# yell/boltzmann-machines

Hardware: AMD Instinct MI355X
Metric: Gibbs-steps/sec (CD-k, 784x1024 RBM, batch 512) (higher is better)
Workload: dtype f32

## Files before the change

### boltzmann_machines_amd/_ffi.py

```python
import ctypes as C
import os

import numpy as np

from . import build as _build

MAX_LAYERS = 4
UNIT_BERNOULLI, UNIT_GAUSSIAN, UNIT_MULTINOMIAL = 0, 1, 2


class Bm355Error(RuntimeError):
    pass


class RbmConfig(C.Structure):
    _fields_ = [('n_visible', C.c_int32), ('n_hidden', C.c_int32), ('v_unit', C.c_int32),
                ('sample_v_states', C.c_int32), ('sample_h_states', C.c_int32),
                ('dbm_first', C.c_int32), ('dbm_last', C.c_int32), ('max_batch', C.c_int32),
                ('l2', C.c_float), ('sparsity_target', C.c_float), ('sparsity_cost', C.c_float),
                ('sparsity_damping', C.c_float), ('dropout', C.c_float),
                ('h_unit', C.c_int32), ('n_samples', C.c_int32)]


class DbmConfig(C.Structure):
# ... 31 lines not shown
    'bm_rbm_set_grad_slot': [_vp, _i32],
    'bm_rbm_allreduce_grads_async': [_vp, _vp],
    'bm_rbm_wait_grads': [_vp, _i32],
    'bm_dbm_allreduce_grads': [_vp, _vp],
    'bm_xchg_create': [C.c_int32, C.c_int32, _vp, _sz, C.POINTER(_vp)],
    'bm_xchg_blob_bytes': [],
    'bm_xchg_export': [_vp, _vp],
    'bm_xchg_attach': [_vp, _vp],
    'bm_xchg_destroy': [_vp],
    'bm_xchg_allreduce_sum': [_vp, _vp],
    'bm_xchg_allreduce_max1': [_vp, _vp, _vp],
    'bm_xchg_status': [_vp, C.POINTER(C.c_int32)],
    'bm_xchg_info': [_vp, C.POINTER(C.c_int32), C.POINTER(C.c_int32), C.POINTER(_sz)],
    'bm_rbm_xchg_create': [_vp, C.c_int32, C.c_int32, C.POINTER(_vp)],
    'bm_dbm_xchg_create': [_vp, C.c_int32, C.c_int32, C.POINTER(_vp)],
    'bm_rbm_allreduce_grads_direct': [_vp, _vp],
    'bm_dbm_allreduce_grads_direct': [_vp, _vp],
    'bm_rbm_exchange_apply_direct': [_vp, _vp, _i32, C.c_float, C.c_float],
    'bm_rbm_exchange_gather_dw': [_vp, _vp],
    'bm_dbm_exchange_apply_ok': [_vp, _vp, C.POINTER(_i32)],
    'bm_dbm_exchange_apply_direct': [_vp, _vp, _i32, _i32, C.c_float, C.c_float],
    'bm_dbm_exchange_gather_dw': [_vp, _vp],
    'bm_xchg_set_timeout': [_vp, C.c_double],
    'bm_xchg_set_max_workgroups': [_vp, _i32],
    'bm_dbm_set_xchg': [_vp, _vp],
    'bm_dbm_set_fast_binary': [_vp, _i32],
    'bm_dbm_set_ais_literal': [_vp, _i32],
    'bm_dbm_set_sigmoid_literal': [_vp, _i32],
    'bm_rbm_set_fast_binary': [_vp, _i32],
    'bm_rbm64_create': [C.POINTER(RbmConfig), C.POINTER(C.c_double), C.POINTER(_vp)],
    'bm_rbm64_destroy': [_vp],
    'bm_rbm64_sync': [_vp],
    'bm_rbm64_seed': [_vp, C.c_uint64],
    'bm_rbm64_set_row_offset': [_vp, C.c_int64],
    'bm_rbm64_set_param': [_vp, C.c_char_p, _vp, _sz],
    'bm_rbm64_get_param': [_vp, C.c_char_p, _vp, _sz],
    'bm_rbm64_train_step': [_vp, _vp, C.c_int32, C.c_double, C.c_double, C.c_int32],
    'bm_rbm64_train_step_metrics': [_vp, _vp, C.c_int32, C.c_double, C.c_double, C.c_int32, C.POINTER(C.c_double)],
    'bm_rbm64_transform': [_vp, _vp, C.c_int32, C.c_int32, _vp],
    'bm_rbm64_metrics': [_vp, _vp, C.c_int32, C.c_int32, C.POINTER(C.c_double)],
    'bm_rbm64_free_energy': [_vp, _vp, C.c_int32, C.POINTER(C.c_double)],
    'bm_dbm64_create': [C.POINTER(DbmConfig), C.POINTER(C.c_double), C.POINTER(_vp)],
    'bm_dbm64_destroy': [_vp],
    'bm_dbm64_sync': [_vp],
    'bm_dbm64_seed': [_vp, C.c_uint64],
    'bm_dbm64_set_row_offset': [_vp, C.c_int64, C.c_int64],
    'bm_dbm64_set_param': [_vp, C.c_char_p, _vp, _sz],
    'bm_dbm64_get_param': [_vp, C.c_char_p, _vp, _sz],
    'bm_dbm64_train_step': [_vp, _vp, C.c_double, C.c_double, C.c_int32, C.POINTER(C.c_int32), C.POINTER(C.c_double)],
    'bm_dbm64_metrics': [_vp, _vp, C.c_int32, C.POINTER(C.c_int32), C.POINTER(C.c_double)],
    'bm_dbm64_mean_field': [_vp, _vp, _vp, C.POINTER(C.c_int32)],
    'bm_dbm64_reconstruct': [_vp, _vp, _vp],
    'bm_dbm64_sample_v': [_vp, C.c_int32, _vp],
    'bm_dbm64_ais': [_vp, C.c_int32, C.c_int32, C.c_int32, C.c_uint64, C.c_int64, _vp],
    'bm_dbm64_log_proba': [_vp, _vp, _vp],
    'bm_rbm_create': [C.POINTER(RbmConfig), C.POINTER(_vp)],
    'bm_rbm_destroy': [_vp],
    'bm_rbm_sync': [_vp],
    'bm_rbm_set_param': [_vp, C.c_char_p, _vp, _sz],
    'bm_rbm_get_param': [_vp, C.c_char_p, _vp, _sz],
    'bm_rbm_set_param_dev': [_vp, C.c_char_p, _vp, _sz],
    'bm_rbm_dev_ptr': [_vp, C.c_char_p, C.POINTER(_vp), C.POINTER(_sz)],
    'bm_rbm_seed': [_vp, _u64],
    'bm_rbm_set_row_offset': [_vp, _i64],
    'bm_rbm_train_step': [_vp, _vp, _i32, _f32, _f32, _i32],
    'bm_rbm_train_step_metrics': [_vp, _vp, _i32, _f32, _f32, _i32, _fp],
    'bm_rbm_train_step_metrics_async': [_vp, _vp, _i32, _f32, _f32, _i32],
    'bm_rbm_collect_metrics': [_vp, _fp, _i32, C.POINTER(C.c_int32)],
    'bm_rbm_train_epoch': [_vp, _vp, _i64, _i32, _f32, _f32, _i32],
    'bm_rbm_stage': [_vp, _i32],
    'bm_rbm_get_staged': [_vp, _i32, C.c_char_p, _vp, _sz],
    'bm_rbm_grad_step': [_vp, _vp, _i32, _i32],
    'bm_rbm_apply_step': [_vp, _i32, _f32, _f32],
    'bm_rbm_transform': [_vp, _vp, _i32, _i32, _vp],
    'bm_rbm_metrics': [_vp, _vp, _i32, _i32, _fp],
    'bm_rbm_free_energy': [_vp, _vp, _i32, _fp],
    'bm_rbm_free_energy_rows': [_vp, _vp, _i32, _vp],
    'bm_rbm_ais': [_vp, _i32, _i32, _i32, _vp, _u64, _i64, _vp],
    'bm_rbm_gibbs': [_vp, _vp, _vp, _i32, _i32],
    'bm_rbm_stream': [_vp, C.POINTER(_vp)],
    'bm_rbm_profile': [_vp, _i32],
    'bm_rbm_kernel_times': [_vp, _fp, _ip],
    'bm_rbm_chain_stats': [_vp, C.POINTER(C.c_int64)],
    'bm_rbm_timer_start': [_vp],
    'bm_rbm_timer_stop': [_vp, _fp],
    'bm_rbm_timer_mark': [_vp],
    'bm_rbm_timer_elapsed': [_vp, _fp],
    'bm_dbm_create': [C.POINTER(DbmConfig), C.POINTER(_vp)],
    'bm_dbm_destroy': [_vp],
    'bm_dbm_sync': [_vp],
    'bm_dbm_seed': [_vp, _u64],
    'bm_dbm_set_row_offset': [_vp, _i64, _i64],
    'bm_dbm_set_param': [_vp, C.c_char_p, _vp, _sz],
    'bm_dbm_get_param': [_vp, C.c_char_p, _vp, _sz],
    'bm_dbm_dev_ptr': [_vp, C.c_char_p, C.POINTER(_vp), C.POINTER(_sz)],
    'bm_dbm_train_step': [_vp, _vp, _f32, _f32, _i32, _ip, _fp],
    'bm_dbm_metrics': [_vp, _vp, _i32, _ip, _fp],
    'bm_dbm_grad_step': [_vp, _vp, _i32, _ip],
    'bm_dbm_apply_step': [_vp, _i32, _i32, _f32, _f32],
    'bm_dbm_set_mf_allreduce': [_vp, _vp, _vp],
    'bm_dbm_set_comm': [_vp, _vp],
    'bm_dbm_ais_sharded': [_vp, _vp, _i32, _i32, _i32, _u64, _vp],
    'bm_dbm_ais_sharded_direct': [_vp, _vp, _i32, _i32, _i32, _u64, _vp],
    'bm_dbm_stream': [_vp, C.POINTER(_vp)],
    'bm_dbm_mean_field': [_vp, _vp, _vp, _ip],
    'bm_dbm_reconstruct': [_vp, _vp, _vp],
    'bm_dbm_sample_v': [_vp, _i32, _vp],
    'bm_dbm_ais': [_vp, _i32, _i32, _i32, _u64, _i64, _vp],
    'bm_dbm_log_proba': [_vp, _vp, _vp],
    'bm_dbm_timer_start': [_vp],
    'bm_dbm_timer_stop': [_vp, _fp],
    'bm_dbm_timer_mark': [_vp],
    'bm_dbm_timer_elapsed': [_vp, _fp],
}
_RESTYPE = {'bm_last_error': C.c_char_p, 'bm_version': C.c_char_p}
MF_REDUCE_FN = C.CFUNCTYPE(C.c_float, C.c_float, C.c_void_p)

_lib = None


def load(rebuild=True):
    global _lib
    if _lib is not None:
        return _lib
    path = _build.LIB
    if rebuild and _build.needs_build():
        import shutil
        have_hipcc = bool(shutil.which('hipcc')) or os.path.exists('/opt/rocm/bin/hipcc')
        try:
            _build.build()
        except Exception as e:
            if have_hipcc or not os.path.exists(path):
                raise Bm355Error('libbm355.so could not be built from the current sources: %s' % e)
            import warnings
            warnings.warn('libbm355.so is older than its sources and hipcc is not available; using the existing '
                          'library (%s)' % e)
    if not os.path.exists(path):
        raise Bm355Error('libbm355.so not found at %s (run __graft_entry__.build())' % path)
    lib = C.CDLL(path)
    for name, restype in _RESTYPE.items():
        f = getattr(lib, name)
        f.restype = restype
        f.argtypes = []
    for name, argtypes in SIGNATURES.items():
        f = getattr(lib, name)
        f.restype = C.c_int
        f.argtypes = argtypes
    _lib = lib
    return lib


def check(rc):
    if rc != 0:
        raise Bm355Error(load().bm_last_error().decode('utf-8', 'replace'))


def exported_symbols():
    return sorted(list(SIGNATURES) + list(_RESTYPE))


class DeviceArray(object):

    def __init__(self, shape, dtype=np.float32, ptr=None, owner=None):
        self.shape = tuple(int(s) for s in (shape if hasattr(shape, '__iter__') else (shape,)))
        self.dtype = np.dtype(dtype)
        self.nbytes = int(np.prod(self.shape)) * self.dtype.itemsize
# ... 52 lines not shown
```

### boltzmann_machines_amd/csrc/bm_chain.h

```cpp
#pragma once
#include "bm_kernels.h"

namespace bm {

constexpr int CHAIN_MAXPH = 24;
constexpr int CHAIN_MAXTI = 64;
using GeoChain = GeoAct8;

struct ChainPhase {
    Operand P, Q; int K; int p_xm; int I;
    const float *bias, *sigma;
    float mult, bmult; int kind, sample;
    float *means, *states, *negmeans; int ldo;
    PhiloxKey key; long long row0;
};

struct ChainArgs {
    int nph, J, tiles_j, rounds_cap, dbg;
    unsigned gen;
    unsigned *flags;
    unsigned *claim;
    unsigned *claim_zero;
    int *status;
    long long *stamps;
// ... 88 lines not shown
    while (true) {
        const int r = small_div(n, T);
        if (r >= R) break;
        const int rem = n - r * T;
        int p = 0;
#pragma unroll
        for (int q = 1; q < CHAIN_MAXPH; ++q) p += (q < c.nph && rem >= c.tp0[q]) ? 1 : 0;
        const int ti = rem - c.tp0[p];
        unsigned nxt = 0;
        const ChainPhase &ph = c.ph[p];
        ActArgs a;
        a.P1 = ph.P; a.Q1 = ph.Q; a.K1 = ph.K; a.p_xm = ph.p_xm;
        a.P2 = Operand{nullptr, 0, 0, 0}; a.Q2 = a.P2; a.K2 = 0;
        a.I = ph.I; a.J = c.J;
        a.bias = ph.bias; a.sigma = ph.sigma; a.mult = ph.mult; a.bmult = ph.bmult; a.kind = ph.kind; a.sample = ph.sample;
        a.means = ph.means; a.states = ph.states; a.negmeans = ph.negmeans; a.ldo = ph.ldo;
        a.key = ph.key; a.row0 = ph.row0;
        a.prev = nullptr; a.maxdiff = nullptr; a.maxdiff_blk = nullptr;
        a.rowacc = nullptr; a.beta_a = 0.f; a.beta_b = 0.f; a.rowacc_single = 0; a.rowdot_out = nullptr; a.ld_part = 0;
        a.dot_vec = nullptr; a.dot_mat = nullptr; a.ld_dot = 0;
        a.acc_init = nullptr; a.ld_init = 0; a.skip = nullptr;
        a.chk_ctl = nullptr; a.chk_slots = nullptr; a.chk_n = 0; a.chk_tol = 0.f;
        a.b3 = Bf3Range{}; a.states16 = nullptr; a.ld16 = 0; a.map_xi = 0;
        a.fe_rowacc2 = nullptr; a.fe_flip = nullptr; a.fe_x = nullptr; a.fe_ldx = 0; a.fe_w = nullptr; a.fe_ldw = 0;
        a.fe_zero = nullptr; a.fe_rm = 0; a.fe_key = PhiloxKey{0u, 0u, 0u, 0u};
#ifdef BM_PROBE
        a.dbg = nullptr;
#endif
        unsigned *fl = c.flags + ((size_t)(team * c.rounds_cap + r) * CHAIN_MAXPH) * CHAIN_MAXTI;
        const unsigned *wfl = (p > 0 && !(c.dbg & 2)) ? fl + (size_t)(p - 1) * CHAIN_MAXTI : nullptr;
        const int nwait = p > 0 ? c.tp0[p] - c.tp0[p - 1] : 0;
        const int tj = team + 8 * r;
        long long *stp = c.stamps ? c.stamps + ((size_t)blockIdx.x * 16 + (ntiles < 15 ? ntiles : 15)) * 8 : nullptr;
        if (stp && tid == 0) { stp[0] = wall_clock64(); stp[5] = (long long)p; stp[6] = (long long)ti; stp[7] = (long long)team; }
        if (ph.p_xm) chain_tile<G, XM, COH>(a, ti * G::TI, tj * G::TJ, smem, wfl, nwait, c.gen, c.status, stp, c.dbg & 4, my_claim, nxt);
        else         chain_tile<G, KM, COH>(a, ti * G::TI, tj * G::TJ, smem, wfl, nwait, c.gen, c.status, stp, c.dbg & 4, my_claim, nxt);
        asm volatile("s_waitcnt vmcnt(0)" ::: "memory");
        if (tid == 0) s_claim = nxt;
        wg_barrier();
        if (tid == 0) __hip_atomic_store(fl + (size_t)p * CHAIN_MAXTI + ti, c.gen, __ATOMIC_RELAXED, __HIP_MEMORY_SCOPE_AGENT);
        if (stp && tid == 0) stp[4] = wall_clock64();
        n = (int)s_claim;
        ++ntiles;
    }
    if (tid == 0 && ntiles) atomicAdd(c.status + 1, ntiles);
}

struct ChainState {
    unsigned *flags = nullptr, *claim = nullptr;
    int *status = nullptr;
    int rounds_cap = 0;
    unsigned gen = 0;
    unsigned launches = 0;
    long long tiles_expected = 0;
    bool on = false;
    int mode = -1;
    int ncu = 0;
    std::vector<ActArgs> rec;
    std::vector<Operand> alt_p;
    long long *stamps = nullptr;
    static constexpr int CLAIM_SLOTS = 16;
    static constexpr size_t STAMP_WORDS = 256 * 16 * 8;
    ChainState() = default;
    ChainState(const ChainState &) = delete;
    ChainState &operator=(const ChainState &) = delete;
    ~ChainState() { release(); }
    void release() {
        if (stamps) {
            const char *f = bm::dbg("chain_stamps");
            std::vector<long long> hst(STAMP_WORDS);
            if (f && hipMemcpy(hst.data(), stamps, STAMP_WORDS * 8, hipMemcpyDeviceToHost) == hipSuccess) {
                FILE *fp = fopen(f, "wb");
                if (fp) { fwrite(hst.data(), 8, STAMP_WORDS, fp); fclose(fp); }
            }
            (void)hipFree(stamps); stamps = nullptr;
        }
        if (flags) (void)hipFree(flags);
        if (claim) (void)hipFree(claim);
        if (status) (void)hipFree(status);
        flags = claim = nullptr; status = nullptr;
    }
};

static inline int chain_mode(ChainState &cs) {
    if (cs.mode < 0) {
        const char *e = bm::dbg("chain");
        cs.mode = e ? atoi(e) : 1;
        hipDeviceProp_t pr; int d = 0, nxcc = 0; (void)hipGetDevice(&d);
        const bool have = hipGetDeviceProperties(&pr, d) == hipSuccess;
        cs.ncu = have ? pr.multiProcessorCount : 0;
        if (hipDeviceGetAttribute(&nxcc, hipDeviceAttributeNumberOfXccs, d) != hipSuccess) nxcc = 0;
        const bool arch = have && (strncmp(pr.gcnArchName, "gfx950", 6) == 0 || strncmp(pr.gcnArchName, "gfx942", 6) == 0);
        if (!(arch && nxcc == 8 && cs.ncu == 256)) cs.mode = 0;
    }
    return cs.mode;
}

static inline bool chain_phase_ok(const ActArgs &a) {
    using G = GeoChain;
    if (a.K2 > 0 || a.b3.K1 > 0 || a.prev || a.maxdiff || a.maxdiff_blk || a.rowacc || a.rowdot_out || a.acc_init ||
        a.skip || a.chk_ctl || a.states16 || a.dot_mat || a.fe_flip) return false;
    if (a.kind != 0 && a.kind != 1) return false;
    const int pl = a.p_xm ? XM : KM;
    if (!(operand_fast(a.P1, pl, a.K1) && operand_fast(a.Q1, XM, a.K1))) return false;
    if (a.K1 < G::PF * G::BK) return false;
    if ((a.I + G::TI - 1) / G::TI > CHAIN_MAXTI) return false;
    return true;
}

static inline int chain_flush(ChainState &cs, hipStream_t st, int maxB) {
    cs.on = false;
    std::vector<ActArgs> rec;
    std::vector<Operand> alt;
    rec.swap(cs.rec);
    alt.swap(cs.alt_p);
    if (rec.empty()) return 0;
    alt.resize(rec.size(), Operand{nullptr, 0, 0, 0});
    using G = GeoChain;
    bool ok = chain_mode(cs) > 0 && rec.size() >= (cs.mode == 1 ? 6u : 2u);
    const int J = rec[0].J, tiles_j = (J + G::TJ - 1) / G::TJ;
    for (const ActArgs &a : rec) ok = ok && chain_phase_ok(a) && a.J == J;
    if (ok && cs.mode == 1) {
        ok = tiles_j >= 8;
        for (const ActArgs &a : rec) ok = ok && ((a.I + G::TI - 1) / G::TI) * ((tiles_j + 7) / 8) <= 2 * 32;
    }
    if (!ok) {
        for (size_t i = 0; i < rec.size(); ++i) {
            if (alt[i].ptr) { rec[i].P1 = alt[i]; rec[i].p_xm = 1; }
            launch_act(rec[i], st);
        }
        return 0;
    }
    const int rounds = (tiles_j + 7) / 8;
    if (!cs.flags || rounds > cs.rounds_cap) {
        if (cs.flags) { if (hipStreamSynchronize(st) != hipSuccess) return -1; (void)hipFree(cs.flags); cs.flags = nullptr; }
        const int cap = std::max(rounds, ((maxB + G::TJ - 1) / G::TJ + 7) / 8);
        const size_t nfl = (size_t)8 * cap * CHAIN_MAXPH * CHAIN_MAXTI;
        if (hipMalloc((void **)&cs.flags, nfl * 4) != hipSuccess) return -1;
        if (hipMemsetAsync(cs.flags, 0, nfl * 4, st) != hipSuccess) return -1;
        cs.rounds_cap = cap;
        cs.gen = 0;
        if (!cs.claim) {
            if (hipMalloc((void **)&cs.claim, (size_t)ChainState::CLAIM_SLOTS * 8 * 32 * 4) != hipSuccess) return -1;
            if (hipMemsetAsync(cs.claim, 0, (size_t)ChainState::CLAIM_SLOTS * 8 * 32 * 4, st) != hipSuccess) return -1;
            if (hipMalloc((void **)&cs.status, 2 * sizeof(int)) != hipSuccess) return -1;
            if (hipMemsetAsync(cs.status, 0, 2 * sizeof(int), st) != hipSuccess) return -1;
        }
    }
    for (size_t first = 0; first < rec.size(); first += CHAIN_MAXPH) {
        const int nph = (int)std::min<size_t>(CHAIN_MAXPH, rec.size() - first);
        ChainArgs c;
        memset(&c, 0, sizeof(c));
        c.nph = nph; c.J = J; c.tiles_j = tiles_j; c.rounds_cap = cs.rounds_cap;
        if (++cs.gen == 0) {
            if (hipMemsetAsync(cs.flags, 0, (size_t)8 * cs.rounds_cap * CHAIN_MAXPH * CHAIN_MAXTI * 4, st) != hipSuccess) return -1;
            cs.gen = 1;
        }
        c.gen = cs.gen;
        c.flags = cs.flags;
        c.claim = cs.claim + (size_t)(cs.launches % ChainState::CLAIM_SLOTS) * 8 * 32;
        c.claim_zero = cs.claim + (size_t)((cs.launches + ChainState::CLAIM_SLOTS / 2) % ChainState::CLAIM_SLOTS) * 8 * 32;
        ++cs.launches;
        c.status = cs.status;
        int tiles = 0;
        for (int p = 0; p < nph; ++p) {
            const ActArgs &a = rec[first + p];
            ChainPhase &ph = c.ph[p];
            ph.P = a.P1; ph.Q = a.Q1; ph.K = a.K1; ph.p_xm = a.p_xm; ph.I = a.I;
            ph.bias = a.bias; ph.sigma = a.sigma; ph.mult = a.mult; ph.bmult = a.bmult; ph.kind = a.kind; ph.sample = a.sample;
            ph.means = a.means; ph.states = a.states; ph.negmeans = a.negmeans; ph.ldo = a.ldo;
            ph.key = a.key; ph.row0 = a.row0;
            c.tp0[p] = tiles;
            tiles += (a.I + G::TI - 1) / G::TI;
        }
        for (int p = nph; p <= CHAIN_MAXPH; ++p) c.tp0[p] = tiles;
        cs.tiles_expected += (long long)tiles * tiles_j;
// ... 13 lines not shown
```

### boltzmann_machines_amd/csrc/bm_gemm.h

```cpp
#pragma once
#include <hip/hip_runtime.h>
#include <stdint.h>
#include <stdlib.h>
#include <string.h>

namespace bm {

struct NoSide {
    static constexpr bool kFinalSync = true;
    static constexpr bool kSplitFill = false, kCohQ = false;
    static constexpr bool kCanAbort = false;
    __device__ __forceinline__ void wait_inputs() {}
    __device__ __forceinline__ void post_fill() {}
    __device__ __forceinline__ void fill() {}
    __device__ __forceinline__ void drain() {}
};

#define BM_ABL(bit) ((ABL >> (bit)) & 1)

typedef float f32x4 __attribute__((ext_vector_type(4)));
typedef float f32x2v __attribute__((ext_vector_type(2)));

constexpr int NT = 256;

enum : int { KM = 0, XM = 1 };

template <int WI_, int WJ_, int MI_, int NJ_, int BK_, int NB_ = 4>
struct Geo {
    static constexpr int WI = WI_, WJ = WJ_, MI = MI_, NJ = NJ_, BK = BK_;
    static constexpr int NBUF = NB_;
    static constexpr int PF = NB_ - 1;
    static constexpr int NW = WI * WJ;
    static constexpr int NT = 64 * NW;
    static constexpr int TI = 16 * MI * WI;
    static constexpr int TJ = 16 * NJ * WJ;
    static constexpr int E = 4 * MI;
    static constexpr int P_BUF = TI * BK;
    static constexpr int Q_BUF = TJ * BK;
    static constexpr int SMEM_FLOATS = NBUF * (P_BUF + Q_BUF);
    static constexpr int NPP = P_BUF * 4 / (1024 * NW);
    static constexpr int NPQ = Q_BUF * 4 / (1024 * NW);
    static constexpr int NVP = TI * BK / (4 * NT);
    static constexpr int NVQ = TJ * BK / (4 * NT);
    static constexpr int SP = (MI == 2) ? 8 : 4;
    static constexpr int SQ = (NJ == 2) ? 8 : 4;
    static_assert(MI == 1 || MI == 2, "MI");
    static_assert(NJ == 1 || NJ == 2, "NJ");
    static_assert(BK == 32 || BK == 64, "BK");
    static_assert(NB_ >= 4 && NB_ <= 8, "ring depth");
    static_assert(NPP >= 1 && NPP * 1024 * NW == P_BUF * 4, "P chunk must split into whole DMA pieces per wave");
    static_assert(NPQ >= 1 && NPQ * 1024 * NW == Q_BUF * 4, "Q chunk must split into whole DMA pieces per wave");
    static_assert(NVP >= 1 && NVP * 4 * NT == TI * BK && NVQ >= 1 && NVQ * 4 * NT == TJ * BK, "register path split");
    static_assert(SMEM_FLOATS * 4 <= 160 * 1024 - 1024, "LDS");
};
using GeoAct = Geo<2, 2, 2, 1, 64>;
using GeoAct8 = Geo<2, 4, 1, 1, 64>;
using GeoActS = Geo<2, 2, 1, 1, 64>;
using GeoActS32 = Geo<2, 2, 1, 1, 32>;
using GeoAct32 = Geo<2, 2, 2, 1, 32>;
using GeoGrad = Geo<2, 2, 2, 2, 64>;
using GeoGrad8 = Geo<2, 4, 2, 1, 64>;
using GeoGrad8h = Geo<2, 4, 2, 1, 32>;
using GeoBf3S = Geo<1, 4, 2, 1, 64>;

struct Operand {
    const float *ptr;
    int ld;
    int nx;
    int vec;
};

static inline Operand make_operand(const float *p, int ld, int nx) {
    Operand o;
    o.ptr = p; o.ld = ld; o.nx = nx;
    o.vec = (((uintptr_t)p & 15u) == 0 && (ld & 3) == 0) ? 1 : 0;
    return o;
}

static inline bool operand_fast(const Operand &o, int layout, int K) {
    if (!o.ptr) return true;
    if (!o.vec) return false;
    return layout == KM ? (o.nx % 4 == 0 && o.nx >= 4) : (K % 4 == 0);
}

template <int BK> __device__ __forceinline__ int fx(int row) { return (BK == 64) ? (row & 15) : ((row >> 1) & 7); }
template <int S> __device__ __forceinline__ int fk(int row) { return S * ((row >> 2) & 1); }

template <int L, int TX, int BK, int S>
__device__ __forceinline__ int img_off(int row, int c4) {
    return (L == XM) ? row * BK + ((c4 ^ fx<BK>(row)) << 2) : row * TX + ((c4 ^ fk<S>(row)) << 2);
}

__device__ __forceinline__ float4 load4_guard(const float *p, bool row_ok, int col, int ncols, bool vec) {
    float4 v = make_float4(0.f, 0.f, 0.f, 0.f);
    if (row_ok) {
// ... 150 lines not shown
}

template <class G, int ABL = 0>
__device__ __forceinline__ void mfma_frags_head(f32x4 (&acc)[G::MI][G::NJ], const Frags<G> &f, int nq) {
#pragma unroll
    for (int q = 0; q < G::BK / 16; ++q) {
        if (q < nq) {
#pragma unroll
            for (int kk = 4 * q; kk < 4 * q + 4; ++kk) {
#pragma unroll
                for (int n = 0; n < G::NJ; ++n) {
                    const float qv = f.q[kk][n];
#pragma unroll
                    for (int t = 0; t < G::MI; ++t) {
                        if (BM_ABL(1)) { acc[t][n][0] += f.p[kk][t] * qv; continue; }
                        acc[t][n] = __builtin_amdgcn_mfma_f32_16x16x4f32(f.p[kk][t], qv, acc[t][n], 0, 0, 0);
                    }
                }
            }
        }
    }
}

template <class G> struct ChunkRegs {
    float4 p[G::NVP];
    float4 q[G::NVQ];
};

struct KRange {
    Operand P1, Q1; int K1;
    Operand P2, Q2; int K2;
};

__device__ __forceinline__ int sel_i(int a, int b, int m) { return a ^ ((a ^ b) & m); }
__device__ __forceinline__ const float *sel_p(const float *a, const float *b, int m) {
    const uintptr_t ua = (uintptr_t)a, ub = (uintptr_t)b;
    return (const float *)(ua ^ ((ua ^ ub) & (uintptr_t)(intptr_t)m));
}

template <class G, int DW = G::NW> struct DmaPlan {
    static constexpr int NPP = G::P_BUF / (256 * DW), NPQ = G::Q_BUF / (256 * DW);
    uint32_t p[NPP], q[NPQ];
};

template <int L, int TX, int BK, int NW, int NP, int S>
__device__ __forceinline__ void plan_offsets(uint32_t (&off)[NP], int ld, int nx, int x0, int wave, int lane) {
    constexpr int RC = (L == KM) ? TX / 4 : BK / 4;
    constexpr int R = 64 / RC;
#pragma unroll
    for (int n = 0; n < NP; ++n) {
        const int pc = wave + n * NW;
        const int row = pc * R + lane / RC, slot = lane % RC;
        if (L == KM) {
            const int c4 = slot ^ fk<S>(row);
            off[n] = (uint32_t)(row * ld + min(x0 + c4 * 4, nx - 4)) * 4u;
        } else {
            const int c4 = slot ^ fx<BK>(row);
            off[n] = (uint32_t)(min(x0 + row, nx - 1) * ld + c4 * 4) * 4u;
        }
    }
}

template <int QL, class G, int PL = KM, int DW = G::NW>
__device__ __forceinline__ void make_plan(DmaPlan<G, DW> &pl, const Operand &P, const Operand &Q, int i0, int j0, int wave, int lane) {
    plan_offsets<PL, G::TI, G::BK, DW, DmaPlan<G, DW>::NPP, G::SP>(pl.p, P.ld, P.nx, i0, wave, lane);
    plan_offsets<QL, G::TJ, G::BK, DW, DmaPlan<G, DW>::NPQ, G::SQ>(pl.q, Q.ld, Q.nx, j0, wave, lane);
}

__device__ __forceinline__ void dma16(const char *src, float *lds_dst) {
    unsigned keep;
    const unsigned lds_addr = (unsigned)(uintptr_t)(__attribute__((address_space(3))) void *)lds_dst;
    asm volatile("s_mov_b32 %0, m0\n\ts_mov_b32 m0, %2\n\ts_nop 0\n\tglobal_load_lds_dwordx4 %1, off\n\ts_mov_b32 m0, %0"
                 : "=&s"(keep) : "v"(src), "s"(__builtin_amdgcn_readfirstlane(lds_addr)) : "memory");
}

__device__ __forceinline__ void dma16s(const void *sbase, uint32_t voff, unsigned lds_byte) {
    asm volatile("s_mov_b32 m0, %2\n\ts_nop 0\n\tglobal_load_lds_dwordx4 %1, %0"
                 :: "s"(sbase), "v"(voff), "s"(lds_byte) : "memory");
}
__device__ __forceinline__ void dma16s_coh(const void *sbase, uint32_t voff, unsigned lds_byte) {
    asm volatile("s_mov_b32 m0, %2\n\ts_nop 0\n\tglobal_load_lds_dwordx4 %1, %0 sc1"
                 :: "s"(sbase), "v"(voff), "s"(lds_byte) : "memory");
}
template <class G, int DW, bool QSC = false, bool QHALF = false>
__device__ __forceinline__ void dma_chunk_s(const DmaPlan<G, DW> &pl, const char *pb, const char *qb, unsigned ldsP, unsigned ldsQ) {
#pragma unroll
    for (int n = 0; n < DmaPlan<G, DW>::NPP; ++n) dma16s(pb, pl.p[n], ldsP + (unsigned)(n * DW * 1024));
#pragma unroll
    for (int n = 0; n < DmaPlan<G, DW>::NPQ; ++n) {
        if (QHALF && (n & 1)) continue;
        if (QSC) dma16s_coh(qb, pl.q[n], ldsQ + (unsigned)(n * DW * 1024));
        else     dma16s(qb, pl.q[n], ldsQ + (unsigned)(n * DW * 1024));
    }
}

template <int QL, class G, bool SEG2, int PL = KM, int DW = G::NW, bool QHALF = false>
__device__ __forceinline__ void dma_chunk(const KRange &kr, const DmaPlan<G, DW> &pl1, const DmaPlan<G, DW> &pl2, int nch1, int c,
                                          float *sP, float *sQ, int wave) {
    constexpr int BK = G::BK;
    const int m = SEG2 ? -(int)(c >= nch1) : 0;
    const int kc = c - (nch1 & m);
    const int ldp = SEG2 ? sel_i(kr.P1.ld, kr.P2.ld, m) : kr.P1.ld;
    const int ldq = SEG2 ? sel_i(kr.Q1.ld, kr.Q2.ld, m) : kr.Q1.ld;
    const char *pb = (const char *)((SEG2 ? sel_p(kr.P1.ptr, kr.P2.ptr, m) : kr.P1.ptr) +
                                    ((PL == KM) ? (size_t)kc * BK * ldp : (size_t)kc * BK));
    const char *qb = (const char *)((SEG2 ? sel_p(kr.Q1.ptr, kr.Q2.ptr, m) : kr.Q1.ptr) +
                                    ((QL == KM) ? (size_t)kc * BK * ldq : (size_t)kc * BK));
#pragma unroll
    for (int n = 0; n < DmaPlan<G, DW>::NPP; ++n) {
        const uint32_t o1 = pl1.p[n], o2 = SEG2 ? pl2.p[n] : 0u;
        const uint32_t o = SEG2 ? (o1 ^ ((o1 ^ o2) & (uint32_t)m)) : o1;
        dma16(pb + o, sP + (wave + n * DW) * 256);
    }
#pragma unroll
    for (int n = 0; n < DmaPlan<G, DW>::NPQ; ++n) {
        if (QHALF && (n & 1)) continue;
        const uint32_t o1 = pl1.q[n], o2 = SEG2 ? pl2.q[n] : 0u;
        const uint32_t o = SEG2 ? (o1 ^ ((o1 ^ o2) & (uint32_t)m)) : o1;
        dma16(qb + o, sQ + (wave + n * DW) * 256);
    }
}

template <int QL, class G, bool FAST, bool SEG2, int PL = KM, bool COHQ = false>
__device__ __forceinline__ void load_chunk(ChunkRegs<G> &r, const KRange &kr, int nch1, int i0, int j0, int c, int tid) {
    constexpr int BK = G::BK;
    if (!SEG2) {
        g2r<PL, G::TI, BK, G::NT, FAST>(r.p, kr.P1.ptr, kr.P1.ld, kr.P1.nx, kr.P1.vec, i0, c * BK, kr.K1, tid);
        g2r<QL, G::TJ, BK, G::NT, FAST, COHQ>(r.q, kr.Q1.ptr, kr.Q1.ld, kr.Q1.nx, kr.Q1.vec, j0, c * BK, kr.K1, tid);
    } else {
        const int m = -(int)((c >= nch1) & (kr.K2 > 0));
        const int kc = c - (nch1 & m);
        const int K = sel_i(kr.K1, kr.K2, m);
        g2r<PL, G::TI, BK, G::NT, FAST>(r.p, sel_p(kr.P1.ptr, kr.P2.ptr, m), sel_i(kr.P1.ld, kr.P2.ld, m),
                                        sel_i(kr.P1.nx, kr.P2.nx, m), sel_i(kr.P1.vec, kr.P2.vec, m), i0, kc * BK, K, tid);
        g2r<QL, G::TJ, BK, G::NT, FAST, COHQ>(r.q, sel_p(kr.Q1.ptr, kr.Q2.ptr, m), sel_i(kr.Q1.ld, kr.Q2.ld, m),
                                              sel_i(kr.Q1.nx, kr.Q2.nx, m), sel_i(kr.Q1.vec, kr.Q2.vec, m), j0, kc * BK, K, tid);
    }
}

template <int QL, class G, bool SEG2, int PL = KM>
__device__ __forceinline__ void store_chunk(const ChunkRegs<G> &r, const KRange &kr, int nch1, int c,
                                            float *sP, float *sQ, int tid) {
    constexpr int BK = G::BK;
    const int m = SEG2 ? -(int)((c >= nch1) & (kr.K2 > 0)) : 0;
    const int kz = sel_i(kr.K1, kr.K2, m) - (c - (nch1 & m)) * BK;
    r2s<PL, G::TI, BK, G::NT, G::SP>(r.p, sP, tid, kz);
    r2s<QL, G::TJ, BK, G::NT, G::SQ>(r.q, sQ, tid, kz);
}

template <class G> struct RegPlan {
    uint32_t p[G::NVP], q[G::NVQ];
};
template <int L, int TX, int BK, int NTH>
__device__ __forceinline__ void reg_offsets(uint32_t (&off)[TX * BK / (4 * NTH)], int ld, int nx, int x0, int tid) {
    constexpr int NV = TX * BK / (4 * NTH);
    constexpr int RC = (L == KM) ? TX / 4 : BK / 4;
#pragma unroll
    for (int n = 0; n < NV; ++n) {
        const int f = tid + n * NTH;
        const int row = f / RC, c4 = f % RC;
        off[n] = (L == KM) ? (uint32_t)(row * ld + min(x0 + c4 * 4, nx - 4)) * 4u
                           : (uint32_t)(min(x0 + row, nx - 1) * ld + c4 * 4) * 4u;
    }
}
template <int QL, class G, int PL = KM>
__device__ __forceinline__ void make_reg_plan(RegPlan<G> &pl, const Operand &P, const Operand &Q, int i0, int j0, int tid) {
    reg_offsets<PL, G::TI, G::BK, G::NT>(pl.p, P.ld, P.nx, i0, tid);
    reg_offsets<QL, G::TJ, G::BK, G::NT>(pl.q, Q.ld, Q.nx, j0, tid);
}
template <int QL, class G, bool SEG2, int PL = KM>
__device__ __forceinline__ void load_chunk_slim(ChunkRegs<G> &r, const KRange &kr, const RegPlan<G> &pl1,
                                                const RegPlan<G> &pl2, int nch1, int c) {
    constexpr int BK = G::BK;
    const int m = SEG2 ? -(int)(c >= nch1) : 0;
    const int kc = c - (nch1 & m);
    const int ldp = SEG2 ? sel_i(kr.P1.ld, kr.P2.ld, m) : kr.P1.ld;
    const int ldq = SEG2 ? sel_i(kr.Q1.ld, kr.Q2.ld, m) : kr.Q1.ld;
    const char *pb = (const char *)((SEG2 ? sel_p(kr.P1.ptr, kr.P2.ptr, m) : kr.P1.ptr) +
                                    ((PL == KM) ? (size_t)kc * BK * ldp : (size_t)kc * BK));
    const char *qb = (const char *)((SEG2 ? sel_p(kr.Q1.ptr, kr.Q2.ptr, m) : kr.Q1.ptr) +
                                    ((QL == KM) ? (size_t)kc * BK * ldq : (size_t)kc * BK));
#pragma unroll
    for (int n = 0; n < G::NVP; ++n) {
        const uint32_t o1 = pl1.p[n], o2 = SEG2 ? pl2.p[n] : 0u;
        const uint32_t o = SEG2 ? (o1 ^ ((o1 ^ o2) & (uint32_t)m)) : o1;
        r.p[n] = *reinterpret_cast<const float4 *>(pb + o);
    }
#pragma unroll
    for (int n = 0; n < G::NVQ; ++n) {
        const uint32_t o1 = pl1.q[n], o2 = SEG2 ? pl2.q[n] : 0u;
        const uint32_t o = SEG2 ? (o1 ^ ((o1 ^ o2) & (uint32_t)m)) : o1;
        r.q[n] = *reinterpret_cast<const float4 *>(qb + o);
    }
}
template <int QL, class G, int PL = KM>
__device__ __forceinline__ void store_chunk_slim(const ChunkRegs<G> &r, float *sP, float *sQ, int tid) {
    r2s<PL, G::TI, G::BK, G::NT, G::SP, false>(r.p, sP, tid, 0);
    r2s<QL, G::TJ, G::BK, G::NT, G::SQ, false>(r.q, sQ, tid, 0);
}

enum : int { STG_DMA = 0, STG_REG = 1, STG_DMAH = 2 };

#define BM_WAIT_VM(n) asm volatile("s_waitcnt vmcnt(%0)" ::"n"(n) : "memory")
template <int NPW, int MAXC>
__device__ __forceinline__ void wait_vm_chunks(int n) {
    static_assert(MAXC * NPW <= 63, "vmcnt range");
    if (MAXC >= 4 && n >= 4)      BM_WAIT_VM(4 * NPW <= 63 ? 4 * NPW : 0);
    else if (MAXC >= 3 && n == 3) BM_WAIT_VM(3 * NPW <= 63 ? 3 * NPW : 0);
    else if (MAXC >= 2 && n == 2) BM_WAIT_VM(2 * NPW <= 63 ? 2 * NPW : 0);
    else if (n == 1)              BM_WAIT_VM(NPW);
    else                          BM_WAIT_VM(0);
}
__device__ __forceinline__ void wg_barrier() {
    asm volatile("s_waitcnt lgkmcnt(0)" ::: "memory");
    __builtin_amdgcn_s_barrier();
    asm volatile("" ::: "memory");
}

template <int QL, class G, bool FAST, bool SEG2, int ABL = 0, int PL = KM, int STG = STG_DMA, class Side = NoSide>
__device__ __forceinline__ void mainloop(f32x4 (&acc)[G::MI][G::NJ], const KRange &kr, int i0, int j0, float *smem,
                                         Side &side, long long *stamps = nullptr) {
#ifdef BM_PROBE
#define BM_MSTAMP(n) do { if (stamps && threadIdx.x == 0) stamps[n] = (long long)__builtin_readcyclecounter(); } while (0)
#else
#define BM_MSTAMP(n) do {} while (0)
#endif
    constexpr int BK = G::BK, P_BUF = G::P_BUF, Q_BUF = G::Q_BUF, NBUF = G::NBUF, PF = G::PF;
    constexpr int DW = (STG == STG_DMAH && G::NW == 8) ? 4 : G::NW;
    constexpr int NPW = DmaPlan<G, DW>::NPP + (BM_ABL(9) ? (DmaPlan<G, DW>::NPQ + 1) / 2 : DmaPlan<G, DW>::NPQ);
    const int tid = threadIdx.x, lane = tid & 63;
    const int w = __builtin_amdgcn_readfirstlane(tid >> 6);
    const int wi = w % G::WI, wj = w / G::WI;
    float *sP = smem, *sQ = smem + NBUF * P_BUF;
    const int nch1 = (kr.K1 + BK - 1) / BK;
    const int nch = nch1 + (SEG2 ? (kr.K2 + BK - 1) / BK : 0);
    const int nfull1 = kr.K1 / BK, nfull2 = SEG2 ? kr.K2 / BK : 0;
    auto is_full = [&](int c) -> bool {
        return (c < nfull1) | (SEG2 && c >= nch1 && c - nch1 < nfull2);
    };
    auto is_dma = [&](int c) -> bool {
        if (!FAST || STG == STG_REG || BM_ABL(6)) return false;
        return is_full(c);
    };
    ChunkRegs<G> gr;
    Frags<G> fa, fb;
    DmaPlan<G, DW> pl1, pl2;
    RegPlan<G> rp1, rp2;
    const bool dmaw = (DW == G::NW) || w < DW;
    ChunkRegs<G> g0, g1;
    if (FAST && STG != STG_REG && dmaw) {
        make_plan<QL, G, PL, DW>(pl1, kr.P1, kr.Q1, i0, j0, w, lane);
        if (SEG2) make_plan<QL, G, PL, DW>(pl2, kr.P2, kr.Q2, i0, j0, w, lane);
    }
    int n_reg = 0;
    if (FAST && STG == STG_REG && !BM_ABL(6) && !BM_ABL(0)) {
        while (n_reg + 4 < nch && is_full(n_reg + 4) && is_full(n_reg + 2)) ++n_reg;
        n_reg &= ~1;
        if (n_reg > 0 && !(is_full(0) && is_full(1) && is_full(2) && is_full(3))) n_reg = 0;
        if (n_reg > 0) {
            make_reg_plan<QL, G, PL>(rp1, kr.P1, kr.Q1, i0, j0, tid);
            if (SEG2) make_reg_plan<QL, G, PL>(rp2, kr.P2, kr.Q2, i0, j0, tid);
        }
    }
    BM_MSTAMP(0);
    if (n_reg > 0) {
        ChunkRegs<G> ga, gb;
        load_chunk_slim<QL, G, SEG2, PL>(ga, kr, rp1, rp2, nch1, 0);
        load_chunk_slim<QL, G, SEG2, PL>(gb, kr, rp1, rp2, nch1, 1);
        load_chunk_slim<QL, G, SEG2, PL>(g0, kr, rp1, rp2, nch1, 2);
        load_chunk_slim<QL, G, SEG2, PL>(g1, kr, rp1, rp2, nch1, 3);
        __builtin_amdgcn_sched_barrier(0);
        side.fill();
        __builtin_amdgcn_sched_barrier(0);
        store_chunk_slim<QL, G, PL>(ga, sP, sQ, tid);
        store_chunk_slim<QL, G, PL>(gb, sP + P_BUF, sQ + Q_BUF, tid);
    } else if constexpr (Side::kSplitFill) {
        static_assert(FAST && STG == STG_DMA && DW == G::NW, "chained fill");
        const unsigned l0 = (unsigned)(uintptr_t)(__attribute__((address_space(3))) void *)smem;
        const unsigned lP = l0 + (unsigned)w * 1024u, lQ = l0 + (unsigned)(NBUF * P_BUF * 4) + (unsigned)w * 1024u;
#pragma unroll
        for (int c = 0; c < PF; ++c) {
            const char *pb = (const char *)kr.P1.ptr + (size_t)c * ((PL == KM) ? (size_t)BK * kr.P1.ld * 4 : (size_t)BK * 4);
#pragma unroll
            for (int n = 0; n < DmaPlan<G, DW>::NPP; ++n) dma16s(pb, pl1.p[n], lP + (unsigned)(c * P_BUF * 4 + n * DW * 1024));
        }
        __builtin_amdgcn_sched_barrier(0);
        side.fill();
        __builtin_amdgcn_sched_barrier(0);
        side.wait_inputs();
#pragma unroll
        for (int c = 0; c < PF; ++c) {
            const char *qb = (const char *)kr.Q1.ptr + (size_t)c * ((QL == KM) ? (size_t)BK * kr.Q1.ld * 4 : (size_t)BK * 4);
#pragma unroll
            for (int n = 0; n < DmaPlan<G, DW>::NPQ; ++n) dma16s_coh(qb, pl1.q[n], lQ + (unsigned)(c * Q_BUF * 4 + n * DW * 1024));
        }
        constexpr int NQ_LEFT = (PF - 2) * DmaPlan<G, DW>::NPQ;
        BM_WAIT_VM(NQ_LEFT);
    } else {
#pragma unroll
        for (int c = 0; c < PF; ++c)
            if (c < nch && is_dma(c) && dmaw && !BM_ABL(0))
                dma_chunk<QL, G, SEG2, PL, DW, (BM_ABL(9) != 0)>(kr, pl1, pl2, nch1, c, sP + (c % NBUF) * P_BUF, sQ + (c % NBUF) * Q_BUF, w);
        __builtin_amdgcn_sched_barrier(0);
        side.fill();
        __builtin_amdgcn_sched_barrier(0);
#pragma unroll
        for (int c = 0; c < 2; ++c)
            if (c < nch && !is_dma(c) && !BM_ABL(0)) {
                load_chunk<QL, G, FAST, SEG2, PL>(gr, kr, nch1, i0, j0, c, tid);
                store_chunk<QL, G, SEG2, PL>(gr, kr, nch1, c, sP + (c % NBUF) * P_BUF, sQ + (c % NBUF) * Q_BUF, tid);
            }
        {
            int n_after = 0;
#pragma unroll
            for (int c = 2; c < PF; ++c) n_after += (c < nch && is_dma(c) && !BM_ABL(0)) ? 1 : 0;
            wait_vm_chunks<NPW, PF - 2>(n_after);
        }
    }
    BM_MSTAMP(1);
    if (!BM_ABL(5)) wg_barrier();
    if constexpr (Side::kCanAbort) {
        side.post_fill();
        if (side.aborted) { BM_WAIT_VM(0); return; }
    }
    read_frags<QL, G, ABL, PL>(fa, sP, sQ, wi, wj, lane);
    BM_MSTAMP(2);
    const int klast = (SEG2 && kr.K2 > 0) ? kr.K2 - (nch - nch1 - 1) * BK : kr.K1 - (nch1 - 1) * BK;
    const int nq_last = (klast + 15) / 16;
    constexpr int NM = (BK / 4) * G::MI * G::NJ;
    constexpr int NRP = (PL == XM) ? BK / 16 : BK / 4;
    constexpr int NRQ = (QL == XM) ? (BK / 16) * G::NJ : BK / 4;
    constexpr int NR = NRP + NRQ;
#define BM_SG(mask, n) __builtin_amdgcn_sched_group_barrier(mask, n, 0);
#ifndef BM_SCHED_VARIANT
#define BM_SCHED_VARIANT 0
#endif
#if BM_SCHED_VARIANT == 0
#define BM_SCHED_STEP                                                                             \
    if (DW == G::NW) { _Pragma("unroll") for (int s_ = 0; s_ < NPW; ++s_) { BM_SG(0x008, 1) BM_SG(0x020, 1) } } \
    _Pragma("unroll") for (int s_ = 0; s_ < NR; ++s_) { BM_SG(0x008, 1) BM_SG(0x100, 1) }         \
    BM_SG(0x008, NM)
#elif BM_SCHED_VARIANT == 1
#define BM_SCHED_STEP                                                                             \
    _Pragma("unroll") for (int s_ = 0; s_ < NR; ++s_) { BM_SG(0x008, 1) BM_SG(0x100, 1) }         \
    _Pragma("unroll") for (int s_ = 0; s_ < NPW; ++s_) { BM_SG(0x008, 1) BM_SG(0x020, 1) }        \
    BM_SG(0x008, NM)
#else
#define BM_SCHED_STEP
#endif
    static_assert(NBUF == 4, "the steps below are written for a 4-slot ring");
    int cc = 0;
    const unsigned lds0 = (unsigned)(uintptr_t)(__attribute__((address_space(3))) void *)smem;
    const unsigned ldsPw = lds0 + (unsigned)w * 1024u, ldsQw = lds0 + (unsigned)(NBUF * P_BUF * 4) + (unsigned)w * 1024u;
    bool in2 = false;
    auto chunk_bases = [&](int c, const char *&pb, const char *&qb) {
        const bool s2 = SEG2 && c >= nch1;
        const Operand &P = s2 ? kr.P2 : kr.P1, &Q = s2 ? kr.Q2 : kr.Q1;
        const int kc = s2 ? c - nch1 : c;
        pb = (const char *)P.ptr + (size_t)kc * ((PL == KM) ? (size_t)BK * P.ld * 4 : (size_t)BK * 4);
        qb = (const char *)Q.ptr + (size_t)kc * ((QL == KM) ? (size_t)BK * Q.ld * 4 : (size_t)BK * 4);
    };
#define BM_DMA_AT(CD, SD)                                                                         \
    {                                                                                             \
        if (SEG2 && !in2 && (CD) >= nch1) { in2 = true; pl1 = pl2; }                              \
        const char *pb_, *qb_;                                                                    \
        chunk_bases((CD), pb_, qb_);                                                              \
        if (dmaw) dma_chunk_s<G, DW, Side::kCohQ, (BM_ABL(9) != 0)>(pl1, pb_, qb_, ldsPw + (unsigned)((SD) * P_BUF * 4), \
                                     ldsQw + (unsigned)((SD) * Q_BUF * 4));                       \
    }
#define BM_STEP_Q(FC, FN, S)                                                                      \
    {                                                                                             \
        BM_DMA_AT(cc + PF, ((S) + PF) % NBUF)                                                     \
        read_frags<QL, G, ABL, PL>(FN, sP + (((S) + 1) % NBUF) * P_BUF, sQ + (((S) + 1) % NBUF) * Q_BUF, wi, wj, lane); \
        mfma_frags<G, ABL>(acc, FC);                                                              \
        BM_SCHED_STEP                                                                             \
        if (!BM_ABL(8)) BM_WAIT_VM((PF - 2) * NPW);                                               \
        if (!BM_ABL(5)) wg_barrier();                                                             \
        ++cc;                                                                                     \
    }
#define BM_STEP_T(FC, FN, S1, S2, S3)       \
    {                                                                                             \
        const int cd = cc + PF, cr = cc + 2;                                                      \
        const bool do_dma = cd < nch && is_dma(cd) && !BM_ABL(0);                                 \
        const bool do_reg = cr < nch && !is_dma(cr) && !BM_ABL(0);                                \
        if (cc == last - 1) side.drain();       \
        if (do_reg) load_chunk<QL, G, FAST, SEG2, PL, Side::kCohQ>(gr, kr, nch1, i0, j0, cr, tid); \
        if (do_dma) BM_DMA_AT(cd, S3)                                                             \
        read_frags<QL, G, ABL, PL>(FN, sP + (S1) * P_BUF, sQ + (S1) * Q_BUF, wi, wj, lane);       \
        mfma_frags<G, ABL>(acc, FC);                                                              \
        _Pragma("unroll") for (int s_ = 0; s_ < NR; ++s_) { BM_SG(0x008, 1) BM_SG(0x100, 1) }     \
        BM_SG(0x008, NM)                                                                          \
        if (do_reg) {                                                                             \
            BM_WAIT_VM(0);                                                                        \
            store_chunk<QL, G, SEG2, PL>(gr, kr, nch1, cr, sP + (S2) * P_BUF, sQ + (S2) * Q_BUF, tid); \
        } else if (cr < nch) {                                                                    \
             \
            int n_after = 0;                                                                      \
            _Pragma("unroll") for (int c_ = 3; c_ <= PF; ++c_) n_after += (cc + c_ < nch && is_dma(cc + c_) && !BM_ABL(0)) ? 1 : 0; \
            wait_vm_chunks<NPW, PF - 2>(n_after);                                                 \
        }                                                                                         \
        if (!BM_ABL(5)) wg_barrier();                                                             \
        ++cc;                                                                                     \
    }
#define BM_STEP_TC(FC, FN, S) BM_STEP_T(FC, FN, ((S) + 1) % NBUF, ((S) + 2) % NBUF, ((S) + 3) % NBUF)
#define BM_STEP_TR(FC, FN)    BM_STEP_T(FC, FN, (cc + 1) % NBUF, (cc + 2) % NBUF, (cc + 3) % NBUF)
    constexpr int NWR = G::NVP + G::NVQ;
#ifndef BM_REG_SCHED_VARIANT
#define BM_REG_SCHED_VARIANT 0
#endif
#if BM_REG_SCHED_VARIANT == 0
#define BM_REG_SCHED(RELOAD)                                                                      \
        _Pragma("unroll") for (int s_ = 0; s_ < NWR; ++s_) { BM_SG(0x008, 1) BM_SG(0x200, 1) }    \
        if (RELOAD) { _Pragma("unroll") for (int s_ = 0; s_ < NWR; ++s_) { BM_SG(0x008, 1) BM_SG(0x020, 1) } } \
        _Pragma("unroll") for (int s_ = 0; s_ < NR; ++s_) { BM_SG(0x008, 1) BM_SG(0x100, 1) }     \
        BM_SG(0x008, NM)
#elif BM_REG_SCHED_VARIANT == 1
#define BM_REG_SCHED(RELOAD)                                                                      \
        _Pragma("unroll") for (int s_ = 0; s_ < NR; ++s_) { BM_SG(0x008, (NM >= 64 ? 2 : 1)) BM_SG(0x100, 2) } \
        _Pragma("unroll") for (int s_ = 0; s_ < NWR; ++s_) { BM_SG(0x008, (NM >= 32 ? 2 : 1)) BM_SG(0x200, 1) } \
        if (RELOAD) { _Pragma("unroll") for (int s_ = 0; s_ < NWR; ++s_) { BM_SG(0x008, 1) BM_SG(0x020, 1) } } \
        BM_SG(0x008, NM)
#else
#define BM_REG_SCHED(RELOAD)
#endif
#define BM_STEP_REG(FC, FN, G_, RELOAD, S)                                                        \
    {                                                                                             \
        store_chunk_slim<QL, G, PL>(G_, sP + (((S) + 2) % NBUF) * P_BUF, sQ + (((S) + 2) % NBUF) * Q_BUF, tid); \
        if (RELOAD) load_chunk_slim<QL, G, SEG2, PL>(G_, kr, rp1, rp2, nch1, cc + 4);             \
        read_frags<QL, G, ABL, PL>(FN, sP + (((S) + 1) % NBUF) * P_BUF, sQ + (((S) + 1) % NBUF) * Q_BUF, wi, wj, lane); \
        mfma_frags<G, ABL>(acc, FC);                                                              \
        BM_REG_SCHED(RELOAD)                                                                      \
        if (!BM_ABL(5)) wg_barrier();                                                             \
        ++cc;                                                                                     \
    }
    if (n_reg > 0) {
        int left = n_reg;
#pragma unroll 1
        while (left >= 4) {
            BM_STEP_REG(fa, fb, g0, true, 0)
            BM_STEP_REG(fb, fa, g1, true, 1)
            BM_STEP_REG(fa, fb, g0, true, 2)
            BM_STEP_REG(fb, fa, g1, true, 3)
            left -= 4;
        }
        if (left == 2) {
            BM_STEP_REG(fa, fb, g0, true, 0)
            BM_STEP_REG(fb, fa, g1, true, 1)
            BM_STEP_REG(fa, fb, g0, false, 2)
            BM_STEP_REG(fb, fa, g1, false, 3)
        } else {
            BM_STEP_REG(fa, fb, g0, false, 0)
            BM_STEP_REG(fb, fa, g1, false, 1)
        }
    }
    int n_steady = 0;
    if (FAST && STG != STG_REG && !BM_ABL(6) && !BM_ABL(0))
        while (n_steady + PF < nch) {
            bool all = true;
#pragma unroll
            for (int c_ = 2; c_ <= PF; ++c_) all = all && is_dma(n_steady + c_);
            if (!all) break;
            ++n_steady;
        }
#pragma unroll 1
    for (int q = 0; q < n_steady / 4; ++q) {
        BM_STEP_Q(fa, fb, 0)
        BM_STEP_Q(fb, fa, 1)
        BM_STEP_Q(fa, fb, 2)
        BM_STEP_Q(fb, fa, 3)
// ... 170 lines not shown
```

### boltzmann_machines_amd/csrc/bm_kernels.h

```cpp
#pragma once
#include <stdio.h>
#include <stdlib.h>
#include <string.h>
#include "bm_gemm.h"
#include "bm_bf3.h"
#include "bm_numerics.h"
#include "bm_rng.h"

namespace bm {

struct MfCtl { unsigned maxdiff; int done; int steps; float resid; };

struct ActArgs {
    Operand P1, Q1; int K1;
    int p_xm;
    Operand P2, Q2; int K2;
    int I, J;
    const float *bias;
    const float *sigma;
    float mult;
    float bmult;
    int kind;
    int sample;
    int lit;
// ... 44 lines not shown
    uint32_t w[4];
    philox_block(key, idx >> 2, w);
    return (int)(w[idx & 3] % (uint32_t)V);
}
#define FE_FLIP_FROM_KEY (reinterpret_cast<const int *>(uintptr_t(1)))
constexpr int BM_MF_SLOTS = 1024;

__device__ __forceinline__ void draw4(const ActArgs &a, const PhiloxKey &key, unsigned long long flat, int ib, int nvalid,
                                      const float *m, float *s, bool aligned) {
    if (aligned) {
        uint32_t wds[4];
        philox_block(key, flat >> 2, wds);
        if (a.kind == 0) {
#pragma unroll
            for (int r = 0; r < 4; ++r) s[r] = (u32_to_uniform(wds[r]) < m[r]) ? 1.f : 0.f;
        } else {
            float n[4];
            box_muller(wds[0], wds[1], n[0], n[1]);
            box_muller(wds[2], wds[3], n[2], n[3]);
#pragma unroll
            for (int r = 0; r < 4; ++r) s[r] = n[r] * a.sigma[ib + r] + m[r];
        }
    } else {
#pragma unroll
        for (int r = 0; r < 4; ++r) {
            if (r >= nvalid) break;
            const unsigned long long idx = flat + r;
            uint32_t wds[4];
            philox_block(key, idx >> 2, wds);
            if (a.kind == 0) {
                s[r] = (u32_to_uniform(wds[idx & 3]) < m[r]) ? 1.f : 0.f;
            } else {
                float n0, n1;
                const int pr = (int)(idx & 3) >> 1;
                box_muller(wds[2 * pr], wds[2 * pr + 1], n0, n1);
                s[r] = ((idx & 1) ? n1 : n0) * a.sigma[ib + r] + m[r];
            }
        }
    }
}

#ifndef BM_NT_STORES
#define BM_NT_STORES 1
#endif
typedef float f32x2 __attribute__((ext_vector_type(2)));
__device__ __forceinline__ void stream_store4(float *p, float x, float y, float z, float w) {
    if (BM_NT_STORES) __builtin_nontemporal_store((f32x4){x, y, z, w}, reinterpret_cast<f32x4 *>(p));
    else *reinterpret_cast<float4 *>(p) = make_float4(x, y, z, w);
}
__device__ __forceinline__ void stream_store2(float *p, float x, float y) {
    if (BM_NT_STORES) __builtin_nontemporal_store((f32x2){x, y}, reinterpret_cast<f32x2 *>(p));
    else *reinterpret_cast<float2 *>(p) = make_float2(x, y);
}

template <bool CACHED = false>
__device__ __forceinline__ void store4(float *dst, size_t o, const float *v, int nvalid, bool v4) {
    if (v4) {
        if (CACHED) *reinterpret_cast<float4 *>(dst + o) = make_float4(v[0], v[1], v[2], v[3]);
        else stream_store4(dst + o, v[0], v[1], v[2], v[3]);
    } else {
#pragma unroll
        for (int r = 0; r < 4; ++r) if (r < nvalid) dst[o + r] = v[r];
    }
}

template <int MI> struct PhiloxFor { typedef PhiloxPair type; };
template <> struct PhiloxFor<1> { typedef PhiloxOne type; };

__device__ __forceinline__ float wave_max_lane63(float v) {
#define BM_DPP_MAX(ctrl, rmask) v = fmaxf(v, __int_as_float(__builtin_amdgcn_update_dpp(__float_as_int(v), __float_as_int(v), ctrl, rmask, 0xf, false)))
    BM_DPP_MAX(0xb1, 0xf);
    BM_DPP_MAX(0x4e, 0xf);
    BM_DPP_MAX(0x124, 0xf);
    BM_DPP_MAX(0x128, 0xf);
    BM_DPP_MAX(0x142, 0xa);
    BM_DPP_MAX(0x143, 0xc);
#undef BM_DPP_MAX
    return v;
}

template <int E, class Rng, bool MF = false, int NTH = 256> struct ActSide {
    static constexpr bool kFinalSync = false;
    static constexpr bool kSplitFill = false, kCohQ = false, kCanAbort = MF;
    static constexpr bool kMF = MF;
    const float *bias, *sigma;
    const float *prev_row;
    int ib0, I, with_rng;
    float bs[E], sg[E], pv[E];
    Rng rng;
    MfCtl *chk_ctl; const float *chk_slots; int chk_n; float chk_tol; const int *skip; float *s_chk; int aborted, nthreads;

    __device__ __forceinline__ void load_inputs() {
        const float *sp = sigma ? sigma : bias;
        const bool has_sigma = sigma != nullptr;
        if (MF && prev_row) {
            if (E == 4 && ib0 + 3 < I && (((uintptr_t)prev_row & 15u) == 0)) {
                const float4 t = *reinterpret_cast<const float4 *>(prev_row);
                pv[0] = t.x; pv[1] = t.y; pv[2] = t.z; pv[E - 1] = t.w;
            } else {
#pragma unroll
                for (int e = 0; e < E; ++e) pv[e] = (ib0 + e < I) ? prev_row[e] : 0.f;
            }
        }
        if (MF && E == 4 && ib0 + 3 < I && (((uintptr_t)(bias + ib0) & 15u) == 0) && (((uintptr_t)(sp + ib0) & 15u) == 0)) {
            const float4 b = *reinterpret_cast<const float4 *>(bias + ib0), v = *reinterpret_cast<const float4 *>(sp + ib0);
            bs[0] = b.x; bs[1] = b.y; bs[2] = b.z; bs[E - 1] = b.w;
            sg[0] = has_sigma ? v.x : 1.0f; sg[1] = has_sigma ? v.y : 1.0f; sg[2] = has_sigma ? v.z : 1.0f; sg[E - 1] = has_sigma ? v.w : 1.0f;
            return;
        }
#pragma unroll
        for (int e = 0; e < E; ++e) {
            const int i = (ib0 + e < I) ? ib0 + e : I - 1;
            bs[e] = bias[i];
            const float sv = sp[i];
            sg[e] = has_sigma ? sv : 1.0f;
        }
    }
    static constexpr int CHK_MAX = 4096;
    float *s_slots;
    static __device__ __forceinline__ void dma4_lane0(const void *src, float *lds_dst) {
        if ((threadIdx.x & 63) == 0) {
            unsigned keep;
            const unsigned lds_addr = (unsigned)(uintptr_t)(__attribute__((address_space(3))) void *)lds_dst;
            asm volatile("s_mov_b32 %0, m0\n\ts_mov_b32 m0, %2\n\ts_nop 0\n\tglobal_load_lds_dword %1, off\n\ts_mov_b32 m0, %0"
                         : "=&s"(keep) : "v"(src), "s"(__builtin_amdgcn_readfirstlane(lds_addr)) : "memory");
        }
    }
    __device__ __forceinline__ void preload() {
        if constexpr (MF) {
            load_inputs();
            aborted = 0;
            const int w = threadIdx.x >> 6, lane = threadIdx.x & 63;
            if (chk_ctl) {
                for (int p = w; p * 256 < chk_n && p * 256 < CHK_MAX; p += nthreads / 64)
                    dma16(reinterpret_cast<const char *>(chk_slots + 256 * p) + 16 * lane, s_slots + 256 * p);
                if (w == 0) dma4_lane0(&chk_ctl->done, s_slots + CHK_MAX);
            } else if (skip) {
                if (w == 0) dma4_lane0(skip, s_slots + CHK_MAX);
            }
        }
    }
    __device__ __forceinline__ void fill() {
        if (!MF) load_inputs();
        if (with_rng) rng.fill();
    }
    __device__ __forceinline__ void post_fill() {
        if constexpr (MF) {
            if (chk_ctl) {
                constexpr int NR = CHK_MAX / (4 * NTH);
                f32x4 v[NR];
#pragma unroll
                for (int q = 0; q < NR; ++q) {
                    const int e = 4 * ((int)threadIdx.x + q * NTH);
                    v[q] = *reinterpret_cast<const f32x4 *>(s_slots + (e < chk_n ? e : 0));
                }
                float m = 0.f;
#pragma unroll
                for (int q = 0; q < NR; ++q) {
                    const bool in = 4 * ((int)threadIdx.x + q * NTH) < chk_n;
                    m = fmaxf(m, in ? fmaxf(fmaxf(v[q][0], v[q][1]), fmaxf(v[q][2], v[q][3])) : 0.f);
                }
                m = wave_max_lane63(m);
                if ((threadIdx.x & 63) == 63) s_chk[threadIdx.x >> 6] = m;
                wg_barrier();
                m = 0.f;
#pragma unroll
// ... 433 lines not shown
                    a.u.vb[c] = a.u.vb[c] + d;
                }
            }
        }
    } else {
        const int c0 = (wv - nv) * 64;
        block_colsum(a.h0m, a.ldh0, a.hm, a.ldh, c0, a.u.H, a.B, true, smem, s1, s2, a.hm_negated != 0);
        if ((lane & 15) == 0) {
#pragma unroll
            for (int r = 0; r < 4; ++r) {
                const int h = c0 + w * 16 + g * 4 + r;
                if (h < a.u.H) {
                    const float sq = s2[r];
                    a.raw_tail[a.u.V + h] = s1[r];
                    a.raw_tail[a.u.V + a.u.H + h] = sq;
                    if (a.raw_only) continue;
                    const float qn = a.u.damping * a.u.q[h] + (1.0f - a.u.damping) * sq;
                    a.u.q[h] = qn;
                    const float pen = a.u.cost * (qn - a.u.target);
                    a.u.pen[h] = pen;
                    float gr = s1[r] / a.u.N;
                    gr = gr - pen;
                    const float d = a.u.lr * (a.u.mom * a.u.dhb[h] + gr);
                    a.u.dhb[h] = d;
                    a.u.hb[h] = a.u.hb[h] + d;
                }
            }
        }
    }
}

__global__ __launch_bounds__(NT) void rbm_bias_fused_kernel(RbmBiasFusedArgs a) {
    __shared__ __attribute__((aligned(16))) float smem[CS_SMEM_FLOATS];
    rbm_bias_fused_block(a, blockIdx.x, smem);
}

struct GradArgs {
    Operand Ppos, Qpos; int Kpos;
    Operand Pneg, Qneg; int Kneg;
    int I, J;
    int form;
    int fused;
    float *raw;
    float *raw2;
    float *W, *dW;
    float *Wt;
    int ldw, ldwt;
    const float *pen;
    float N, M, l2, lr, mom;
    int nbias;
    RbmBiasFusedArgs bias;
    int fetch_at_fill;
    int map_xi;
#ifdef BM_PROBE
    long long *dbg;
#endif
};

__device__ __forceinline__ void apply_w_update(float g, float pen, float l2, float lr, float mom,
                                               float &w, float &dw) {
    g = __fsub_rn(g, __fmul_rn(l2, w));
    g = __fsub_rn(g, pen);
    const float d = __fmul_rn(lr, __fadd_rn(__fmul_rn(mom, dw), g));
    dw = d;
    w = __fadd_rn(w, d);
}
__device__ __forceinline__ bool grad_pow2(float N) { return ((__float_as_uint(N) & 0x007fffffu) == 0u) && N >= 1.0f; }
__device__ __forceinline__ float grad_norm1(float r, float N, float invN, bool pow2) {
    return pow2 ? __fmul_rn(r, invN) : __fdiv_rn(r, N);
}
__device__ __forceinline__ float grad_norm2(float r, float r2, float N, float M, float invN, float invM, bool pow2) {
    return pow2 ? __fsub_rn(__fmul_rn(r, invN), __fmul_rn(r2, invM)) : __fsub_rn(__fdiv_rn(r, N), __fdiv_rn(r2, M));
}

struct DivBy {
    float n, inv; bool pow2;
    __device__ __forceinline__ explicit DivBy(float N) : n(N), inv(1.0f / N),
        pow2(grad_pow2(N)) {}
};

template <int NJ> struct GradSide {
    static constexpr bool kFinalSync = true;
    static constexpr bool kSplitFill = false, kCohQ = false, kCanAbort = false;
    const float *W, *dW; int ldw, I, J, ib0, jb[NJ]; bool on, vec8;
    float4 w[NJ][2], d[NJ][2];
    bool at_fill;
    __device__ __forceinline__ void fill() { if (at_fill) fetch(); }
    __device__ __forceinline__ void drain() { if (!at_fill) fetch(); }
    __device__ __forceinline__ void fetch() {
        if (!on || ib0 >= I) return;
#pragma unroll
        for (int n = 0; n < NJ; ++n) {
            if (jb[n] >= J) continue;
            const size_t o = (size_t)jb[n] * ldw + ib0;
            if (vec8) {
                w[n][0] = *reinterpret_cast<const float4 *>(W + o);  w[n][1] = *reinterpret_cast<const float4 *>(W + o + 4);
                d[n][0] = *reinterpret_cast<const float4 *>(dW + o); d[n][1] = *reinterpret_cast<const float4 *>(dW + o + 4);
            } else {
                float tw[8], td[8];
#pragma unroll
                for (int e = 0; e < 8; ++e) {
                    const bool ok = ib0 + e < I;
                    tw[e] = ok ? W[o + e] : 0.f;
                    td[e] = ok ? dW[o + e] : 0.f;
                }
                w[n][0] = make_float4(tw[0], tw[1], tw[2], tw[3]); w[n][1] = make_float4(tw[4], tw[5], tw[6], tw[7]);
                d[n][0] = make_float4(td[0], td[1], td[2], td[3]); d[n][1] = make_float4(td[4], td[5], td[6], td[7]);
            }
        }
    }
};

template <class G, bool FAST, int ABL = 0, int STG = STG_DMA, int MINB = 1>
__global__ __launch_bounds__(G::NT, MINB) void grad_kernel(GradArgs a, TileMap tmap) {
    constexpr int TI = G::TI, NJ = G::NJ;
    static_assert(G::MI == 2 && G::TI == 64 && G::TJ == 64, "grad_kernel: 64 x 64 tiles, 8 consecutive outputs per lane");
    __shared__ __attribute__((aligned(16))) float smem[G::SMEM_FLOATS];
    constexpr bool kBias = G::SMEM_FLOATS >= CS_SMEM_FLOATS;
    static_assert(G::NT >= NT, "bias path");
    const int ntile_blocks = (int)gridDim.x - a.nbias;
    if ((int)blockIdx.x >= ntile_blocks) {
        if constexpr (kBias) {
            if (G::NT > NT && threadIdx.x >= NT) return;
            rbm_bias_fused_block(a.bias, (int)blockIdx.x - ntile_blocks, smem);
        }
        return;
    }
    asm volatile("" :: "s"(a.Ppos.ptr), "s"(a.Qpos.ptr), "s"(a.Ppos.ld), "s"(a.Qpos.ld), "s"(a.Ppos.nx), "s"(a.Qpos.nx),
                       "s"(a.Pneg.ptr), "s"(a.Qneg.ptr), "s"(a.Pneg.ld), "s"(a.Qneg.ld), "s"(a.Kpos), "s"(a.Kneg),
                       "s"(a.I), "s"(a.J), "s"(a.W), "s"(a.dW), "s"(a.ldw), "s"(a.form), "s"(a.fused));
    constexpr int TJ2 = G::TJ;
    int ti, tj;
    if (tmap.slab) {
        block_to_tile((a.J + TJ2 - 1) / TJ2, ti, tj, 0, a.nbias);
    } else {
        TILE_WORDS(tmap, (int)blockIdx.x);
        TILE_OF_BLOCK(tmap, (int)blockIdx.x, ntile_blocks, ti, tj);
    }
    const int i0 = ti * TI, j0 = tj * TJ2;
    const int tid = threadIdx.x, lane = tid & 63, w = tid >> 6;
    const int wi = w % G::WI, wj = w / G::WI;
    const int g = lane >> 4, l15 = lane & 15;
    const int ib0 = i0 + wi * 32 + g * 8;

#ifdef BM_PROBE
#define BM_GSTAMP(n) do { if (a.dbg && threadIdx.x == 0) a.dbg[blockIdx.x * 4 + (n)] = (long long)__builtin_readcyclecounter(); } while (0)
#else
#define BM_GSTAMP(n) do {} while (0)
#endif
    BM_GSTAMP(0);
    f32x4 pos[2][NJ], neg[2][NJ];
#pragma unroll
    for (int t = 0; t < 2; ++t)
#pragma unroll
        for (int n = 0; n < NJ; ++n) pos[t][n] = neg[t][n] = (f32x4){0.f, 0.f, 0.f, 0.f};
    GradSide<NJ> side;
    side.W = a.W; side.dW = a.dW; side.ldw = a.ldw; side.I = a.I; side.J = a.J; side.ib0 = ib0;
#pragma unroll
    for (int n = 0; n < NJ; ++n) side.jb[n] = j0 + wj * (16 * NJ) + lane_j<KM, G>(l15, n);
    side.vec8 = (ib0 + 7 < a.I) && ((a.ldw & 3) == 0);
    side.at_fill = true;
    side.on = a.fused != 0 && a.fetch_at_fill != 0;
    KRange kr;
    kr.P1 = a.Ppos; kr.Q1 = a.Qpos; kr.K1 = a.Kpos;
    if (a.form == 0) {
        kr.P2 = a.Pneg; kr.Q2 = a.Qneg; kr.K2 = a.Kneg;
        mainloop<KM, G, FAST, true, ABL, KM, STG>(pos, kr, i0, j0, smem, side);
    } else {
        kr.P2 = a.Ppos; kr.Q2 = a.Qpos; kr.K2 = 0;
        mainloop<KM, G, FAST, false, 0, KM, STG>(pos, kr, i0, j0, smem, side);
        kr.P1 = a.Pneg; kr.Q1 = a.Qneg; kr.K1 = a.Kneg;
        mainloop<KM, G, FAST, false, 0, KM, STG>(neg, kr, i0, j0, smem, side);
    }

    BM_GSTAMP(1);
    if (ib0 >= a.I) return;
    if (!a.fetch_at_fill) { side.on = a.fused != 0; side.fetch(); }
    const DivBy divN(a.N), divM(a.M);
    float wt[NJ][8];
    bool jok[NJ];
#pragma unroll
    for (int n = 0; n < NJ; ++n) {
        const int j = side.jb[n];
        jok[n] = j < a.J;
        if (!jok[n]) continue;
        float pv[8], nv[8];
        lane_outputs<G>(pos, n, pv);
        lane_outputs<G>(neg, n, nv);
        const size_t o = (size_t)j * a.ldw + ib0;
        if (!a.fused) {
#pragma unroll
            for (int e = 0; e < 8; ++e) {
                if (ib0 + e >= a.I) break;
                a.raw[o + e] = pv[e];
                if (a.form != 0) a.raw2[o + e] = nv[e];
            }
            continue;
        }
        float wv[8] = {side.w[n][0].x, side.w[n][0].y, side.w[n][0].z, side.w[n][0].w, side.w[n][1].x, side.w[n][1].y, side.w[n][1].z, side.w[n][1].w};
        float dv[8] = {side.d[n][0].x, side.d[n][0].y, side.d[n][0].z, side.d[n][0].w, side.d[n][1].x, side.d[n][1].y, side.d[n][1].z, side.d[n][1].w};
        float pe[8];
#pragma unroll
        for (int e = 0; e < 8; ++e) pe[e] = (a.pen && ib0 + e < a.I) ? a.pen[ib0 + e] : 0.f;
        float gr[8];
        if (divN.pow2 && divM.pow2) {
#pragma unroll
            for (int e = 0; e < 8; ++e) gr[e] = (a.form == 0) ? grad_norm1(pv[e], a.N, divN.inv, true)
                                                              : grad_norm2(pv[e], nv[e], a.N, a.M, divN.inv, divM.inv, true);
        } else {
#pragma unroll
            for (int e = 0; e < 8; ++e) gr[e] = (a.form == 0) ? grad_norm1(pv[e], a.N, 0.f, false)
                                                              : grad_norm2(pv[e], nv[e], a.N, a.M, 0.f, 0.f, false);
        }
#pragma unroll
        for (int e = 0; e < 8; ++e) {
            apply_w_update(gr[e], pe[e], a.l2, a.lr, a.mom, wv[e], dv[e]);
            wt[n][e] = wv[e];
        }
        if (side.vec8) {
            stream_store4(a.W + o, wv[0], wv[1], wv[2], wv[3]);
            stream_store4(a.W + o + 4, wv[4], wv[5], wv[6], wv[7]);
            stream_store4(a.dW + o, dv[0], dv[1], dv[2], dv[3]);
            stream_store4(a.dW + o + 4, dv[4], dv[5], dv[6], dv[7]);
        } else {
#pragma unroll
            for (int e = 0; e < 8; ++e)
                if (ib0 + e < a.I) { a.W[o + e] = wv[e]; a.dW[o + e] = dv[e]; }
        }
    }
    if (a.fused && a.Wt) {
        const int ja = side.jb[0];
        const bool pair = NJ == 2 && jok[0] && jok[NJ - 1] && ((a.ldwt & 1) == 0);
#pragma unroll
        for (int e = 0; e < 8; ++e) {
            if (ib0 + e >= a.I) break;
            float *dst = a.Wt + (size_t)(ib0 + e) * a.ldwt + ja;
            if (pair) {
                stream_store2(dst, wt[0][e], wt[NJ - 1][e]);
            } else {
                if (jok[0]) dst[0] = wt[0][e];
                if (NJ == 2 && jok[NJ - 1]) dst[1] = wt[NJ - 1][e];
            }
        }
    }
    BM_GSTAMP(2);
}

struct ApplyWArgs {
    const float *raw, *raw2;
    float *W, *dW, *Wt;
    const float *pen;
    int I, J, ldw, ldwt;
    int form;
    float N, M, l2, lr, mom;
};
__global__ void apply_w_kernel(ApplyWArgs a) {
    const size_t n = (size_t)a.I * a.J;
    for (size_t e = (size_t)blockIdx.x * blockDim.x + threadIdx.x; e < n; e += (size_t)gridDim.x * blockDim.x) {
        const int i = (int)(e % (size_t)a.I), j = (int)(e / (size_t)a.I);
        const size_t o = (size_t)j * a.ldw + i;
        const float gr = (a.form == 0) ? grad_norm1(a.raw[o], a.N, 0.f, false) : grad_norm2(a.raw[o], a.raw2[o], a.N, a.M, 0.f, 0.f, false);
        float wv = a.W[o], dv = a.dW[o];
        apply_w_update(gr, a.pen ? a.pen[i] : 0.f, a.l2, a.lr, a.mom, wv, dv);
        a.W[o] = wv;
        a.dW[o] = dv;
        if (a.Wt) a.Wt[(size_t)i * a.ldwt + j] = wv;
    }
}

__device__ __forceinline__ void rbm_bias_update(const RbmBiasArgs &a, int c) {
    if (c < a.V) {
        const float g = a.sv[c] / a.N;
        const float d = a.lr * (a.mom * a.dvb[c] + g);
        a.dvb[c] = d;
        a.vb[c] = a.vb[c] + d;
    } else if (c < a.V + a.H) {
        const int h = c - a.V;
        const float qn = a.damping * a.q[h] + (1.0f - a.damping) * a.sq[h];
        a.q[h] = qn;
        const float pen = a.cost * (qn - a.target);
        a.pen[h] = pen;
        float g = a.sh[h] / a.N;
        g = g - pen;
        const float d = a.lr * (a.mom * a.dhb[h] + g);
        a.dhb[h] = d;
        a.hb[h] = a.hb[h] + d;
    }
}
__global__ __launch_bounds__(256) void apply_w_tiled_kernel(ApplyWArgs a, RbmBiasArgs b, int nbias) {
    __shared__ float tile[64][65];
    const int ntile = (int)gridDim.x - nbias;
    if ((int)blockIdx.x >= ntile) {
        rbm_bias_update(b, ((int)blockIdx.x - ntile) * 256 + (int)threadIdx.x);
        return;
    }
    const int tiles_i = (a.I + 63) / 64;
    const int i0 = ((int)blockIdx.x % tiles_i) * 64, j0 = ((int)blockIdx.x / tiles_i) * 64;
    const int tid = threadIdx.x, c4 = tid & 15, r0 = tid >> 4;
    const bool pow2 = grad_pow2(a.N) && grad_pow2(a.M);
    const float invN = 1.0f / a.N, invM = 1.0f / a.M;
    const int i = i0 + 4 * c4;
    float4 pe = make_float4(0.f, 0.f, 0.f, 0.f);
    if (a.pen && i < a.I) pe = *reinterpret_cast<const float4 *>(a.pen + i);
#pragma unroll
    for (int p = 0; p < 4; ++p) {
        const int jl = r0 + 16 * p, j = j0 + jl;
        if (j < a.J && i < a.I) {
            const size_t o = (size_t)j * a.ldw + i;
            const float4 r = *reinterpret_cast<const float4 *>(a.raw + o);
            float4 wv = *reinterpret_cast<const float4 *>(a.W + o), dv = *reinterpret_cast<const float4 *>(a.dW + o);
            float4 g;
            if (a.form == 0) {
                g = make_float4(grad_norm1(r.x, a.N, invN, pow2), grad_norm1(r.y, a.N, invN, pow2),
                                grad_norm1(r.z, a.N, invN, pow2), grad_norm1(r.w, a.N, invN, pow2));
            } else {
                const float4 r2 = *reinterpret_cast<const float4 *>(a.raw2 + o);
                g = make_float4(grad_norm2(r.x, r2.x, a.N, a.M, invN, invM, pow2), grad_norm2(r.y, r2.y, a.N, a.M, invN, invM, pow2),
                                grad_norm2(r.z, r2.z, a.N, a.M, invN, invM, pow2), grad_norm2(r.w, r2.w, a.N, a.M, invN, invM, pow2));
            }
            apply_w_update(g.x, pe.x, a.l2, a.lr, a.mom, wv.x, dv.x);
            apply_w_update(g.y, pe.y, a.l2, a.lr, a.mom, wv.y, dv.y);
            apply_w_update(g.z, pe.z, a.l2, a.lr, a.mom, wv.z, dv.z);
            apply_w_update(g.w, pe.w, a.l2, a.lr, a.mom, wv.w, dv.w);
            *reinterpret_cast<float4 *>(a.W + o) = wv;
            *reinterpret_cast<float4 *>(a.dW + o) = dv;
            tile[jl][4 * c4] = wv.x; tile[jl][4 * c4 + 1] = wv.y; tile[jl][4 * c4 + 2] = wv.z; tile[jl][4 * c4 + 3] = wv.w;
        }
    }
// ... 680 lines not shown
```

### boltzmann_machines_amd/csrc/bm_rbm.hip

```cpp
#include "../../include/bm355.h"
#include "bm_common.h"
#include "bm_kernels.h"
#include "bm_chain.h"

#include <math.h>
#include <atomic>
#include <memory>

namespace bm {

static thread_local char g_err[1024] = "";
void set_error(const char *fmt, ...) {
    va_list ap;
    va_start(ap, fmt);
    vsnprintf(g_err, sizeof(g_err), fmt, ap);
    va_end(ap);
}

enum : uint32_t { SITE_DROPOUT = 1, SITE_H0 = 2, SITE_V = 3, SITE_H = 4, SITE_PLL = 5, SITE_FE = 6 };
enum : uint32_t { SITE_AIS_V0 = 7, SITE_AIS_V = 8, SITE_AIS_H = 9 };

}

using namespace bm;

struct bm_xchg;
static int xchg_check_status(bm_xchg *x);
static void xchg_bind_user(bm_xchg *x, bm_xchg **slot);
static void xchg_dw_replaced(bm_xchg *x);

struct bm_rbm {
    bm_rbm_config cfg;
    bm_xchg *xchg_used = nullptr;
    bool dw_sharded = false;
    int V, H, maxB;
    Stream stream;
    Stream comm_stream;
    Stream stage_stream;
    Event ev0, ev1;
    Mat W, dW;
    Mat Wt;
    bool use_wt = false, wt_valid = false;
    DevBuf vb, hb, dvb, dhb, q, sigma;
    Mat h0m, h0s, hm, hs, hneg;
    Mat vm, vs, Xs, Xd;
    DevBuf grad;
    DevBuf grad_alt;
    int grad_slot = 0;
    Event ev_ready[2], ev_reduced[2];
    DevBuf pen;
    DevBuf rowacc;
    DevBuf hhat;
    DevArray<int> flip;
    DevArray<double> scal;
    bool multinomial() const { return cfg.h_unit == BM_UNIT_MULTINOMIAL; }
    uint64_t seed = 0;
    uint32_t call = 0;
    int64_t row0 = 0;
    const float *Xin = nullptr;
    int Xin_ld = 0;
    bool hm_is_neg = false;
    bool fe_in_chain = false;
    DevBuf fe_part;
    int ais_rows = 0;
    Mat av, ah;
    DevBuf apart_h, apart_v;
    DevArray<double> alogw;
    DevBuf abase, adot, abeta, atable;
    int fer_rows = 0;
    DevBuf fer_part, fer_out;
    int fast = 0;
    bool fast_now = false;
    Mat16 W3, W3t, hs16, vs16;
    DevArray<int> nonbinary;
    struct Stage { Mat W, dW; DevBuf vb, hb, dvb, dhb, q, sigma; Event ev; bool ready = false;
                   std::atomic<int> readers{0}; } stage[2];
    int last_stage = -1;
    Pinned<float> stage_host;
    int device = 0;
    static constexpr int MRING = 4096;
    Pinned<double> mring;
    double *mring_dev = nullptr;
    std::vector<int> mring_B;
    int mring_n = 0;
    Event ev_mlast;
    bool prof = false;
    struct Rec { int cls; Event a, b; };
    std::vector<Rec> recs;
    size_t grad_tail() const { return (size_t)V * W.ld; }
    ChainState chain;
};

enum { KC_UP = 0, KC_DOWN = 1, KC_GRAD = 2, KC_COLSUM = 3, KC_BIAS = 4, KC_OTHER = 5 };

static int check_dw(const bm_rbm *h, const char *what) {
    BM_CHECK(!h->dw_sharded, "%s: after bm_rbm_exchange_apply_direct this rank holds only its slice of the momentum buffer dW; "
             "every rank must call bm_rbm_exchange_gather_dw first (DirectExchange.gather_dw())", what);
    return 0;
}

struct ProfScope {
    bm_rbm *h; hipEvent_t b = nullptr;
    ProfScope(bm_rbm *h_, int cls) : h(h_) {
        if (!h->prof) return;
        bm_rbm::Rec r{cls};
        (void)create(r.a); (void)create(r.b);
        (void)hipEventRecord(r.a, h->stream);
        b = r.b;
        h->recs.push_back(std::move(r));
    }
    ~ProfScope() { if (b) (void)hipEventRecord(b, h->stream); }
};

static PhiloxKey make_key(const bm_rbm *h, uint32_t site, int t) {
    PhiloxKey k;
    k.k0 = (uint32_t)h->seed;
    k.k1 = (uint32_t)(h->seed >> 32);
    k.site = site + 16u * (uint32_t)t;
    k.call = h->call;
    return k;
}

static void act_pass(bm_rbm *h, const ActArgs &a, const Operand *alt_p = nullptr) {
    if (h->chain.on) {
        h->chain.rec.push_back(a);
        h->chain.alt_p.resize(h->chain.rec.size(), Operand{nullptr, 0, 0, 0});
        if (alt_p) h->chain.alt_p.back() = *alt_p;
    } else if (alt_p) {
        ActArgs b = a;
        b.P1 = *alt_p; b.p_xm = 1;
        launch_act(b, h->stream);
    } else launch_act(a, h->stream);
}
static void chain_begin(bm_rbm *h) {
    h->chain.on = !h->prof && !h->multinomial() && !h->fast_now && chain_mode(h->chain) > 0;
}
static int chain_end(bm_rbm *h) {
    BM_CHECK(chain_flush(h->chain, h->stream, h->maxB) == 0, "chained launch: %s", hipGetErrorString(hipGetLastError()));
    return 0;
}

static void ensure_wt(bm_rbm *h) {
    if (!h->use_wt || h->wt_valid) return;
    const int nt = ((h->V + 31) / 32) * ((h->H + 31) / 32);
    hipLaunchKernelGGL(transpose_kernel, dim3(nt), dim3(256), 0, h->stream, (const float *)h->W.p, h->W.ld, h->Wt.p, h->Wt.ld, h->V, h->H);
    h->wt_valid = true;
}

static void launch_up(bm_rbm *h, const float *v, int ldv, int B, float *means, float *states, int ldo,
                      int sample, uint32_t site, int t, float *negmeans = nullptr, bool fe = false) {
    ProfScope _ps(h, KC_UP);
    ActArgs a;
    memset(&a, 0, sizeof(a));
    a.P1 = make_operand(h->W.p, h->W.ld, h->H);
    a.Q1 = make_operand(v, ldv, B);
    a.K1 = h->V;
    a.I = h->H; a.J = B;
    a.bias = h->hb.p; a.sigma = nullptr;
    a.mult = 1.0f + (h->cfg.dbm_first ? 1.0f : 0.0f);
    a.bmult = a.mult;
    a.kind = BM_UNIT_BERNOULLI;
    a.sample = states ? sample : 0;
    a.means = means; a.states = states; a.negmeans = negmeans; a.ldo = ldo;
    a.key = make_key(h, site, t);
    a.row0 = h->row0;
    if (fe) {
        const int nslot = (h->H + 15) / 16, rm = (nslot + 3) & ~3;
        a.rowacc = h->fe_part.p; a.rowacc_single = 1; a.beta_b = 1.f; a.ld_part = h->maxB; a.fe_rm = rm;
        a.fe_rowacc2 = h->fe_part.p + (size_t)rm * h->maxB;
        a.fe_flip = FE_FLIP_FROM_KEY; a.fe_key = make_key(h, SITE_PLL, 0); a.fe_zero = h->scal.p;
        a.fe_x = v; a.fe_ldx = ldv; a.fe_w = h->W.p; a.fe_ldw = h->W.ld;
    }
    if (h->fast_now && v == h->vs.p) {
        a.b3.P1 = Bf3Operand{h->W3t.p, h->W3t.plane_stride(), h->W3t.ld, h->H};
        a.b3.Q1 = Bf3Operand{h->vs16.p, 0, h->vs16.ld, B};
        a.b3.K1 = h->vs16.ld;
        if (states == h->hs.p) { a.states16 = h->hs16.p; a.ld16 = h->hs16.ld; }
    }
    if (h->multinomial()) {
        if (!means) { means = h->hm.p; ldo = h->hm.ld; }
        a.kind = 3; a.sample = 0; a.means = means; a.ldo = ldo; a.states = nullptr; a.negmeans = nullptr;
        launch_act(a, h->stream);
        SmArgs m;
        memset(&m, 0, sizeof(m));
        m.L = means; m.ld = ldo; m.I = h->H; m.J = B; m.M = h->cfg.n_samples; m.sample = sample;
        m.states = states; m.negmeans = negmeans; m.key = a.key; m.row0 = h->row0;
        hipLaunchKernelGGL(softmax_multinomial_kernel, dim3(B), dim3(64), 2 * (size_t)h->H * sizeof(float), h->stream, m);
        return;
    }
    if (h->use_wt && h->wt_valid && !(h->fast_now && v == h->vs.p)) {
        const Operand wt = make_operand(h->Wt.p, h->Wt.ld, h->H);
        act_pass(h, a, &wt);
    } else act_pass(h, a);
}

static void launch_down(bm_rbm *h, const float *hs, int ldh, int B, float *means, float *states, int ldo,
                        int sample, uint32_t site, int t) {
    ProfScope _ps(h, KC_DOWN);
    ActArgs a;
    memset(&a, 0, sizeof(a));
    a.P1 = make_operand(h->W.p, h->W.ld, h->V);
    a.p_xm = 1;
    a.Q1 = make_operand(hs, ldh, B);
    a.K1 = h->H;
    a.I = h->V; a.J = B;
    a.bias = h->vb.p; a.sigma = h->sigma.p;
    a.mult = 1.0f + (h->cfg.dbm_last ? 1.0f : 0.0f);
    a.bmult = a.mult;
    a.kind = h->cfg.v_unit;
    a.sample = sample;
    a.means = means; a.states = states; a.ldo = ldo;
    a.key = make_key(h, site, t);
    a.row0 = h->row0;
    if (h->fast_now && hs == h->hs.p) {
        a.b3.P1 = Bf3Operand{h->W3.p, h->W3.plane_stride(), h->W3.ld, h->V};
        a.b3.Q1 = Bf3Operand{h->hs16.p, 0, h->hs16.ld, B};
        a.b3.K1 = h->hs16.ld;
        if (states == h->vs.p) { a.states16 = h->vs16.p; a.ld16 = h->vs16.ld; }
    }
    act_pass(h, a);
}

static bool metrics_fused_ok(const bm_rbm *h);
static void metrics_prep(bm_rbm *h, int B);
static int run_chain(bm_rbm *h, const float *X_dev, int B, int k, float *hm_out, bool need_vm = true, bool for_update = false,
                     bool split_step = false, bool fetch = false) {
    BM_CHECK(B >= 1 && B <= h->maxB, "batch %d outside [1, max_batch=%d]", B, h->maxB);
    BM_CHECK(k >= 1, "n_gibbs_steps must be >= 1 (got %d)", k);
    if (!split_step) ensure_wt(h);
    const float *Xin = X_dev;
    int ldx = h->V;
    if (h->cfg.v_unit == BM_UNIT_GAUSSIAN) {
        hipLaunchKernelGGL(div_cols_kernel, dim3(256), dim3(256), 0, h->stream, Xin, ldx, h->sigma.p, h->Xs.p,
                           h->Xs.ld, B, h->V);
        Xin = h->Xs.p; ldx = h->Xs.ld;
    }
    if (h->cfg.dropout >= 0.f) {
        hipLaunchKernelGGL(dropout_kernel, dim3(256), dim3(256), 0, h->stream, Xin, ldx, h->Xd.p, h->Xd.ld, B, h->V,
                           h->cfg.dropout, make_key(h, SITE_DROPOUT, 0),
                           (unsigned long long)h->row0 * (unsigned long long)h->V);
        Xin = h->Xd.p; ldx = h->Xd.ld;
    }
    h->Xin = Xin; h->Xin_ld = ldx;
    const bool fe = fetch && metrics_fused_ok(h);
    if (fe && !h->fe_part.p) BM_TRY(h->fe_part.alloc((size_t)2 * ((((h->H + 15) / 16) + 3) & ~3) * h->maxB));
    h->fe_in_chain = fe;
    if (fetch && !fe) metrics_prep(h, B);
    chain_begin(h);
    launch_up(h, Xin, ldx, B, h->h0m.p, h->h0s.p, h->h0m.ld, 1, SITE_H0, 0, nullptr, fe);
    const float *hstate = h->cfg.sample_h_states ? h->h0s.p : h->h0m.p;
    for (int t = 0; t < k; ++t) {
        const bool last = t == k - 1;
        launch_down(h, hstate, h->hs.ld, B, (need_vm && last) ? h->vm.p : nullptr, h->vs.p, h->vm.ld,
                    h->cfg.sample_v_states, SITE_V, t);
        const bool last_out = hm_out && last;
        const bool neg_only = last && !hm_out && !need_vm && !h->multinomial();
        h->hm_is_neg = neg_only;
        launch_up(h, h->vs.p, h->vs.ld, B, last_out ? hm_out : (neg_only ? nullptr : h->hm.p), last ? nullptr : h->hs.p,
                  last_out ? h->H : h->hm.ld, h->cfg.sample_h_states, SITE_H, t, (!hm_out && last) ? h->hneg.p : nullptr);
        hstate = h->hs.p;
    }
    BM_TRY(chain_end(h));
    return 0;
}

static void fill_bias(bm_rbm *h, float N, float lr, float mom, RbmBiasArgs &b) {
    float *tail = h->grad.p + h->grad_tail();
    b.sv = tail; b.sh = tail + h->V; b.sq = tail + h->V + h->H;
    b.vb = h->vb.p; b.dvb = h->dvb.p; b.hb = h->hb.p; b.dhb = h->dhb.p; b.q = h->q.p; b.pen = h->pen.p;
    b.V = h->V; b.H = h->H;
    b.N = N; b.lr = lr; b.mom = mom;
    b.damping = h->cfg.sparsity_damping; b.cost = h->cfg.sparsity_cost; b.target = h->cfg.sparsity_target;
}

static int fill_bias_fused(bm_rbm *h, int B, float lr, float mom, RbmBiasFusedArgs &a) {
    memset(&a, 0, sizeof(a));
    a.X = h->Xin; a.ldx = h->Xin_ld; a.vs = h->vs.p; a.ldv = h->vs.ld;
    a.h0m = h->h0m.p; a.ldh0 = h->h0m.ld; a.B = B;
    if (h->hm_is_neg) { a.hm = h->hneg.p; a.ldh = h->hneg.ld; a.hm_negated = 1; }
    else              { a.hm = h->hm.p; a.ldh = h->hm.ld; }
    a.raw_tail = h->grad.p + h->grad_tail();
    RbmBiasArgs &b = a.u;
    b.vb = h->vb.p; b.dvb = h->dvb.p; b.hb = h->hb.p; b.dhb = h->dhb.p; b.q = h->q.p; b.pen = h->pen.p;
    b.V = h->V; b.H = h->H;
    b.N = (float)B; b.lr = lr; b.mom = mom;
    b.damping = h->cfg.sparsity_damping; b.cost = h->cfg.sparsity_cost; b.target = h->cfg.sparsity_target;
    return (h->V + 63) / 64 + (h->H + 63) / 64;
}

static void launch_bias_fused(bm_rbm *h, int B, float lr, float mom) {
    ProfScope _ps(h, KC_COLSUM);
    RbmBiasFusedArgs a;
    const int nw = fill_bias_fused(h, B, lr, mom, a);
    hipLaunchKernelGGL(rbm_bias_fused_kernel, dim3(nw), dim3(NT), 0, h->stream, a);
}

static void rbm_grad(bm_rbm *h, int B, int fused, float N, float lr, float mom, bool with_bias);

static void launch_update_fused(bm_rbm *h, int B, float lr, float mom) {
    if (h->cfg.sparsity_cost != 0.f) {
        launch_bias_fused(h, B, lr, mom);
        rbm_grad(h, B, 1, (float)B, lr, mom, false);
    } else {
        rbm_grad(h, B, 1, (float)B, lr, mom, true);
    }
}

static void fill_grad(bm_rbm *h, int B, int fused, float N, float lr, float mom, GradArgs &g) {
    memset(&g, 0, sizeof(g));
    g.Ppos = make_operand(h->h0m.p, h->h0m.ld, h->H);
    g.Qpos = make_operand(h->Xin, h->Xin_ld, h->V);
    g.Kpos = B;
    g.Pneg = make_operand(h->hneg.p, h->hneg.ld, h->H);
    g.Qneg = make_operand(h->vs.p, h->vs.ld, h->V);
    g.Kneg = B;
    g.I = h->H; g.J = h->V;
    g.form = 0; g.fused = fused;
    g.raw = h->grad.p; g.raw2 = nullptr;
    g.W = h->W.p; g.dW = h->dW.p; g.Wt = nullptr;
    g.ldw = h->W.ld; g.ldwt = 0;
    if (h->use_wt && fused) { g.Wt = h->Wt.p; g.ldwt = h->Wt.ld; }
    g.N = N; g.M = N; g.l2 = h->cfg.l2; g.lr = lr; g.mom = mom;
}
static void rbm_grad(bm_rbm *h, int B, int fused, float N, float lr, float mom, bool with_bias) {
    ProfScope _ps(h, KC_GRAD);
    GradArgs g;
    fill_grad(h, B, fused, N, lr, mom, g);
    g.pen = with_bias ? nullptr : h->pen.p;
    if (with_bias) {
        g.nbias = fill_bias_fused(h, B, lr, mom, g.bias);
        g.bias.raw_only = fused ? 0 : 1;
    }
// ... 198 lines not shown
int bm_dev_alloc(size_t bytes, void **out_dev) { BM_HIP(hipMalloc(out_dev, bytes ? bytes : 1)); return 0; }
int bm_dev_free(void *dev) { BM_HIP(hipFree(dev)); return 0; }
int bm_h2d(void *dst, const void *src, size_t bytes) {
    static const bool pin = !(bm::dbg("h2d_pin") && atoi(bm::dbg("h2d_pin")) == 0);
    if (pin && bytes >= ((size_t)32 << 20)) {
        if (hipHostRegister(const_cast<void *>(src), bytes, hipHostRegisterDefault) == hipSuccess) {
            const hipError_t e = hipMemcpy(dst, src, bytes, hipMemcpyHostToDevice);
            (void)hipHostUnregister(const_cast<void *>(src));
            BM_HIP(e);
            return 0;
        }
        (void)hipGetLastError();
    }
    BM_HIP(hipMemcpy(dst, src, bytes, hipMemcpyHostToDevice));
    return 0;
}
int bm_d2h(void *dst, const void *src, size_t bytes) { BM_HIP(hipMemcpy(dst, src, bytes, hipMemcpyDeviceToHost)); return 0; }
int bm_dev_memset(void *dst, int value, size_t bytes) { BM_HIP(hipMemset(dst, value, bytes)); return 0; }

int bm_rbm_create(const bm_rbm_config *cfg, bm_rbm **out) {
    BM_CHECK(cfg && out, "null argument");
    BM_CHECK(cfg->n_visible >= 1 && cfg->n_hidden >= 1, "bad layer sizes %d x %d", cfg->n_visible, cfg->n_hidden);
    BM_CHECK(cfg->max_batch >= 1, "max_batch must be >= 1");
    BM_CHECK(cfg->v_unit == BM_UNIT_BERNOULLI || cfg->v_unit == BM_UNIT_GAUSSIAN, "unknown visible unit %d", cfg->v_unit);
    BM_CHECK(cfg->h_unit == BM_UNIT_BERNOULLI || cfg->h_unit == BM_UNIT_MULTINOMIAL, "unknown hidden unit %d", cfg->h_unit);
    if (cfg->h_unit == BM_UNIT_MULTINOMIAL) {
        BM_CHECK(cfg->n_samples >= 1, "MultinomialRBM: n_samples must be >= 1 (got %d)", cfg->n_samples);
        BM_CHECK(cfg->n_hidden <= 8192, "MultinomialRBM: n_hidden %d > 8192 (softmax row staged in LDS)", cfg->n_hidden);
    }
    BM_CHECK(bm_device_count() > 0, "no HIP device visible: libbm355 has no CPU fallback");
    auto h = std::make_unique<bm_rbm>();
    h->cfg = *cfg;
    h->V = cfg->n_visible; h->H = cfg->n_hidden; h->maxB = cfg->max_batch;
    const int V = h->V, H = h->H, B = h->maxB;
    BM_HIP(hipGetDevice(&h->device));
    BM_TRY(create(h->stream)); BM_TRY(create(h->ev0)); BM_TRY(create(h->ev1));
    BM_TRY(h->W.alloc(V, H)); BM_TRY(h->dW.alloc(V, H));
    {
        const char *e = bm::dbg("up_xm");
        h->use_wt = !(e && atoi(e) == 0) && (V % 4 == 0) && !h->multinomial();
        if (h->use_wt) BM_TRY(h->Wt.alloc(H, V));
    }
    BM_TRY(h->vb.alloc(V)); BM_TRY(h->hb.alloc(H)); BM_TRY(h->dvb.alloc(V)); BM_TRY(h->dhb.alloc(H));
    BM_TRY(h->q.alloc(H)); BM_TRY(h->sigma.alloc(V));
    BM_TRY(h->h0m.alloc(B, H)); BM_TRY(h->h0s.alloc(B, H)); BM_TRY(h->hm.alloc(B, H)); BM_TRY(h->hs.alloc(B, H)); BM_TRY(h->hneg.alloc(B, H));
    BM_TRY(h->vm.alloc(B, V)); BM_TRY(h->vs.alloc(B, V)); BM_TRY(h->Xs.alloc(B, V)); BM_TRY(h->Xd.alloc(B, V));
    BM_TRY(h->grad.alloc(h->grad_tail() + V + 2 * (size_t)H));
    BM_TRY(h->pen.alloc(H));
    BM_TRY(h->rowacc.alloc(3 * (size_t)B)); BM_TRY(h->hhat.alloc(3 * (size_t)H));
    BM_TRY(h->flip.alloc(B)); BM_TRY(h->scal.alloc(6));
    {
        std::vector<float> ones(V, 1.0f);
        BM_HIP(hipMemcpy(h->sigma.p, ones.data(), V * sizeof(float), hipMemcpyHostToDevice));
    }
    *out = h.release();
    return 0;
}

int bm_rbm_destroy(bm_rbm *h) {
    if (!h) return 0;
    for (hipStream_t st : {h->stream.h, h->comm_stream.h, h->stage_stream.h}) if (st) (void)hipStreamSynchronize(st);
    if (h->xchg_used) xchg_bind_user(h->xchg_used, nullptr);
    delete h;
    return 0;
}

static int check_device_status(bm_rbm *h) {
    if (h->xchg_used) BM_TRY(xchg_check_status(h->xchg_used));
    if (h->chain.status) {
        int st[2] = {0, 0};
        BM_HIP(hipMemcpy(st, h->chain.status, sizeof(st), hipMemcpyDeviceToHost));
        const long long expect = h->chain.tiles_expected & 0xffffffffLL;
        if (st[0] != 0 || (long long)(unsigned)st[1] != expect) {
            h->chain.mode = 0;
            h->chain.tiles_expected = 0;
            BM_HIP(hipMemset(h->chain.status, 0, sizeof(st)));
            BM_CHECK(st[0] == 0, "chained propagation launch failed (status %d: %s); the results since the last check are "
                     "invalid, chained launches are now off for this handle", st[0],
                     st[0] == CHAIN_ERR_TIMEOUT ? "a wait for a producing tile expired" : "not an 8-XCD device");
            BM_CHECK(false, "chained propagation launches computed %u tiles, expected %lld; the results since the last check "
                     "are invalid, chained launches are now off for this handle", (unsigned)st[1], expect);
        }
    }
    return 0;
}

int bm_rbm_sync(bm_rbm *h) {
    BM_HIP(hipStreamSynchronize(h->stream));
    BM_TRY(check_device_status(h));
    if (h->nonbinary.p) {
        int bad = 0;
        BM_HIP(hipMemcpy(&bad, h->nonbinary.p, sizeof(int), hipMemcpyDeviceToHost));
        if (bad) {
            BM_HIP(hipMemset(h->nonbinary.p, 0, sizeof(int)));
            BM_CHECK(false, "fast-binary mode: bm_rbm_gibbs was given hidden states that are not a {0,1} bitmap");
        }
    }
    return 0;
}

int bm_rbm_set_fast_binary(bm_rbm *h, int32_t on) {
    BM_CHECK(h, "null argument");
    h->fast = (on >= 2 || (on == 1 && (long long)h->V * h->H >= (8ll << 20))) ? 1 : 0;
    return 0;
}

static DevBuf *find_vec(bm_rbm *h, const std::string &n) {
    if (n == "vb") return &h->vb;
    if (n == "hb") return &h->hb;
    if (n == "dvb") return &h->dvb;
    if (n == "dhb") return &h->dhb;
    if (n == "q_means") return &h->q;
    if (n == "sigma") return &h->sigma;
    return nullptr;
}

int bm_rbm_set_param(bm_rbm *h, const char *name, const float *host, size_t n) {
    const std::string nm(name ? name : "");
    BM_HIP(hipStreamSynchronize(h->stream));
    if (nm == "W" || nm == "dW") {
        BM_CHECK(n == (size_t)h->V * h->H, "variable '%s' has %zu elements, got %zu", name, (size_t)h->V * h->H, n);
        BM_TRY((nm == "W" ? h->W : h->dW).upload(host));
        if (nm == "W") h->wt_valid = false;
        else { h->dw_sharded = false; if (h->xchg_used) xchg_dw_replaced(h->xchg_used); }
        return 0;
    }
    DevBuf *b = find_vec(h, nm);
    BM_CHECK(b, "unknown RBM variable '%s'", name ? name : "(null)");
    BM_CHECK(n == b->n, "variable '%s' has %zu elements, got %zu", name, b->n, n);
    BM_HIP(hipMemcpy(b->p, host, n * sizeof(float), hipMemcpyHostToDevice));
    return 0;
}

int bm_rbm_set_param_dev(bm_rbm *h, const char *name, const float *src_dev, size_t n) {
    const std::string nm(name ? name : "");
    BM_CHECK(h && src_dev, "null argument");
    if (nm == "W" || nm == "dW") {
        BM_CHECK(n == (size_t)h->V * h->H, "variable '%s' has %zu elements, got %zu", name, (size_t)h->V * h->H, n);
        Mat &m = nm == "W" ? h->W : h->dW;
        if (nm == "W") h->wt_valid = false;
        else { h->dw_sharded = false; if (h->xchg_used) xchg_dw_replaced(h->xchg_used); }
        BM_HIP(hipMemcpy2DAsync(m.p, (size_t)m.ld * sizeof(float), src_dev, (size_t)m.cols * sizeof(float),
                                (size_t)m.cols * sizeof(float), m.rows, hipMemcpyDeviceToDevice, h->stream));
        return 0;
    }
    DevBuf *b = find_vec(h, nm);
    BM_CHECK(b, "unknown RBM variable '%s'", name ? name : "(null)");
    BM_CHECK(n == b->n, "variable '%s' has %zu elements, got %zu", name, b->n, n);
    BM_HIP(hipMemcpyAsync(b->p, src_dev, n * sizeof(float), hipMemcpyDeviceToDevice, h->stream));
    return 0;
}

int bm_rbm_get_param(bm_rbm *h, const char *name, float *host, size_t n) {
    const std::string nm(name ? name : "");
    BM_HIP(hipStreamSynchronize(h->stream));
    BM_TRY(check_device_status(h));
    if (nm == "W" || nm == "dW") {
        BM_CHECK(n == (size_t)h->V * h->H, "variable '%s' has %zu elements, got %zu", name, (size_t)h->V * h->H, n);
        if (nm == "dW") BM_TRY(check_dw(h, "bm_rbm_get_param(dW)"));
        return (nm == "W" ? h->W : h->dW).download(host);
    }
    DevBuf *b = find_vec(h, nm);
    BM_CHECK(b, "unknown RBM variable '%s'", name ? name : "(null)");
    BM_CHECK(n == b->n, "variable '%s' has %zu elements, got %zu", name, b->n, n);
    BM_HIP(hipMemcpy(host, b->p, n * sizeof(float), hipMemcpyDeviceToHost));
    return 0;
}

int bm_rbm_stage(bm_rbm *h, int32_t slot) {
    BM_CHECK(h && (slot == 0 || slot == 1), "bad stage slot %d", (int)slot);
    bm_rbm::Stage &sg = h->stage[slot];
    BM_CHECK(sg.readers.load() == 0, "stage slot %d is being read by bm_rbm_get_staged: use the other slot", (int)slot);
    BM_TRY(check_dw(h, "bm_rbm_stage"));
    if (!sg.ev) {
        BM_TRY(sg.W.alloc(h->V, h->H)); BM_TRY(sg.dW.alloc(h->V, h->H));
        BM_TRY(sg.vb.alloc(h->V)); BM_TRY(sg.dvb.alloc(h->V)); BM_TRY(sg.sigma.alloc(h->V));
        BM_TRY(sg.hb.alloc(h->H)); BM_TRY(sg.dhb.alloc(h->H)); BM_TRY(sg.q.alloc(h->H));
        BM_TRY(create(sg.ev, hipEventDisableTiming));
    }
    if (!h->stage_stream) BM_TRY(create(h->stage_stream, hipStreamNonBlocking));
    static const bool bound = !(bm::dbg("stage_ahead") && atoi(bm::dbg("stage_ahead")) == 0);
    if (bound && h->last_stage >= 0) BM_HIP(hipEventSynchronize(h->stage[h->last_stage].ev));
    BM_HIP(hipMemcpyAsync(sg.W.p, h->W.p, h->W.count() * sizeof(float), hipMemcpyDeviceToDevice, h->stream));
    BM_HIP(hipMemcpyAsync(sg.dW.p, h->dW.p, h->dW.count() * sizeof(float), hipMemcpyDeviceToDevice, h->stream));
    DevBuf *src[] = {&h->vb, &h->hb, &h->dvb, &h->dhb, &h->q, &h->sigma};
    DevBuf *dst[] = {&sg.vb, &sg.hb, &sg.dvb, &sg.dhb, &sg.q, &sg.sigma};
    for (int i = 0; i < 6; ++i)
        BM_HIP(hipMemcpyAsync(dst[i]->p, src[i]->p, src[i]->n * sizeof(float), hipMemcpyDeviceToDevice, h->stream));
    BM_HIP(hipEventRecord(sg.ev, h->stream));
    sg.ready = true;
    h->last_stage = slot;
    return 0;
}
int bm_rbm_get_staged(bm_rbm *h, int32_t slot, const char *name, float *host, size_t n) {
    BM_CHECK(h && (slot == 0 || slot == 1) && h->stage[slot].ready, "stage slot %d holds no snapshot", (int)slot);
    BM_HIP(hipSetDevice(h->device));
    bm_rbm::Stage &sg = h->stage[slot];
    struct Reading { std::atomic<int> &n; Reading(std::atomic<int> &r) : n(r) { ++n; } ~Reading() { --n; } } reading(sg.readers);
    const std::string nm(name ? name : "");
    BM_HIP(hipEventSynchronize(sg.ev));
    const size_t need = (size_t)h->V * h->H * sizeof(float);
    if (!h->stage_host) BM_TRY(create(h->stage_host, (size_t)h->V * h->H));
    if (h->chain.status) {
        BM_HIP(hipMemcpyAsync(h->stage_host, h->chain.status, sizeof(int), hipMemcpyDeviceToHost, h->stage_stream));
        BM_HIP(hipStreamSynchronize(h->stage_stream));
        BM_CHECK(*(const int *)h->stage_host.h == 0, "a chained propagation launch failed (status %d) before this snapshot: "
                 "it is invalid (bm_rbm_sync reports and recovers)", *(const int *)h->stage_host.h);
    }
    if (nm == "W" || nm == "dW") {
        BM_CHECK(n == (size_t)h->V * h->H, "variable '%s' has %zu elements, got %zu", name, (size_t)h->V * h->H, n);
        const Mat &m = nm == "W" ? sg.W : sg.dW;
        BM_HIP(hipMemcpy2DAsync(h->stage_host, (size_t)m.cols * sizeof(float), m.p, (size_t)m.ld * sizeof(float),
                                (size_t)m.cols * sizeof(float), m.rows, hipMemcpyDeviceToHost, h->stage_stream));
    } else {
        const char *names[] = {"vb", "hb", "dvb", "dhb", "q_means", "sigma"};
        DevBuf *bufs[] = {&sg.vb, &sg.hb, &sg.dvb, &sg.dhb, &sg.q, &sg.sigma};
        DevBuf *b = nullptr;
        for (int i = 0; i < 6; ++i) if (nm == names[i]) b = bufs[i];
        BM_CHECK(b, "unknown RBM variable '%s'", name ? name : "(null)");
        BM_CHECK(n == b->n, "variable '%s' has %zu elements, got %zu", name, b->n, n);
        BM_CHECK(n * sizeof(float) <= need, "variable '%s' larger than the bounce buffer", name);
        BM_HIP(hipMemcpyAsync(h->stage_host, b->p, n * sizeof(float), hipMemcpyDeviceToHost, h->stage_stream));
    }
    BM_HIP(hipStreamSynchronize(h->stage_stream));
    memcpy(host, h->stage_host, n * sizeof(float));
    return 0;
}

int bm_rbm_dev_ptr(bm_rbm *h, const char *name, void **out_dev, size_t *out_n) {
    const std::string nm(name ? name : "");
    DevBuf *b = (nm == "grad") ? &h->grad : find_vec(h, nm);
    BM_CHECK(b, "no device view for '%s' (matrices are pitched; use get/set_param)", name ? name : "(null)");
    *out_dev = b->p;
    if (out_n) *out_n = b->n;
    return 0;
}

int bm_rbm_seed(bm_rbm *h, uint64_t seed) { h->seed = seed; h->call = 0; return 0; }
int bm_rbm_set_row_offset(bm_rbm *h, int64_t row0) { h->row0 = row0; return 0; }

int bm_rbm_train_step(bm_rbm *h, const float *X_dev, int32_t B, float lr, float mom, int32_t k) {
    BM_TRY(check_dw(h, "bm_rbm_train_step"));
    BM_TRY(run_chain(h, X_dev, B, k, nullptr, false, true));
    launch_update_fused(h, B, lr, mom);
    h->call++;
    BM_HIP(hipGetLastError());
    return 0;
}

int bm_rbm_train_step_metrics(bm_rbm *h, const float *X_dev, int32_t B, float lr, float mom, int32_t k,
                              float *out4) {
    BM_TRY(check_dw(h, "bm_rbm_train_step_metrics"));
    BM_TRY(run_chain(h, X_dev, B, k, nullptr, true, false, false, true));
    BM_TRY(metrics_from_chain(h, B, out4));
    launch_update_fused(h, B, lr, mom);
    h->call++;
    BM_HIP(hipGetLastError());
    return 0;
}

int bm_rbm_train_step_metrics_async(bm_rbm *h, const float *X_dev, int32_t B, float lr, float mom, int32_t k) {
    if (!h->mring) {
        Pinned<double> ring;
        BM_TRY(create(ring, (size_t)bm_rbm::MRING * 6));
        BM_TRY(create(h->ev_mlast, hipEventDisableTiming));
        BM_HIP(hipHostGetDevicePointer((void **)&h->mring_dev, ring, 0));
        h->mring_B.resize(bm_rbm::MRING);
        h->mring = std::move(ring);
    }
    BM_CHECK(h->mring_n < bm_rbm::MRING, "%d metric fetches are pending: call bm_rbm_collect_metrics", h->mring_n);
    BM_TRY(check_dw(h, "bm_rbm_train_step_metrics_async"));
    BM_TRY(run_chain(h, X_dev, B, k, nullptr, true, false, false, true));
    BM_TRY(metrics_from_chain(h, B, nullptr));
    hipLaunchKernelGGL(scal_to_host_kernel, dim3(1), dim3(64), 0, h->stream, (const double *)h->scal.p,
                       h->mring_dev + (size_t)h->mring_n * 6);
    BM_HIP(hipEventRecord(h->ev_mlast, h->stream));
    h->mring_B[h->mring_n++] = B;
    launch_update_fused(h, B, lr, mom);
    h->call++;
    BM_HIP(hipGetLastError());
    return 0;
}
int bm_rbm_collect_metrics(bm_rbm *h, float *out4n, int32_t max_n, int32_t *out_n) {
    BM_CHECK(h && out_n && (out4n || max_n == 0), "null argument");
    BM_CHECK(h->mring_n <= max_n, "%d fetches pending, room for %d", h->mring_n, (int)max_n);
    if (h->mring_n > 0 && h->ev_mlast) BM_HIP(hipEventSynchronize(h->ev_mlast));
    if (h->chain.status || h->xchg_used) {
        BM_HIP(hipStreamSynchronize(h->stream));
        const int rc = check_device_status(h);
        if (rc) { h->mring_n = 0; *out_n = 0; return rc; }
    }
    for (int i = 0; i < h->mring_n; ++i) metrics_to_out4(h, h->mring + (size_t)i * 6, h->mring_B[i], out4n + 4 * (size_t)i);
    *out_n = h->mring_n;
    h->mring_n = 0;
    return 0;
}

int bm_rbm_train_epoch(bm_rbm *h, const float *X_dev, int64_t N, int32_t batch, float lr, float mom, int32_t k) {
    BM_CHECK(batch >= 1 && N >= 1, "bad N=%lld batch=%d", (long long)N, batch);
    for (int64_t s = 0; s < N; s += batch) {
        const int B = (int)((N - s < batch) ? (N - s) : batch);
        BM_TRY(bm_rbm_train_step(h, X_dev + (size_t)s * h->V, B, lr, mom, k));
    }
    return 0;
}

int bm_rbm_grad_step(bm_rbm *h, const float *X_dev, int32_t B, int32_t k) {
    BM_TRY(run_chain(h, X_dev, B, k, nullptr, false, false, true));
    rbm_grad(h, B, 0, (float)B, 0.f, 0.f, true);
    h->call++;
    BM_HIP(hipGetLastError());
    return 0;
}

static int ensure_delayed(bm_rbm *h) {
    if (h->comm_stream) return 0;
    BM_TRY(h->grad_alt.alloc(h->grad.n));
    for (int i = 0; i < 2; ++i) {
        BM_TRY(create(h->ev_ready[i], hipEventDisableTiming));
        BM_TRY(create(h->ev_reduced[i], hipEventDisableTiming));
    }
    return create(h->comm_stream);
}
int bm_rbm_set_grad_slot(bm_rbm *h, int32_t slot) {
    BM_CHECK(h && (slot == 0 || slot == 1), "slot must be 0 or 1");
    if (slot == h->grad_slot) return 0;
    BM_TRY(ensure_delayed(h));
    std::swap(h->grad, h->grad_alt);
    h->grad_slot = slot;
    return 0;
}
int bm_rbm_allreduce_grads_async(bm_rbm *h, bm_comm *c) {
    BM_CHECK(h && c, "null argument");
    BM_TRY(ensure_delayed(h));
    const int s = h->grad_slot;
    BM_HIP(hipEventRecord(h->ev_ready[s], h->stream));
    BM_HIP(hipStreamWaitEvent(h->comm_stream, h->ev_ready[s], 0));
    BM_TRY(bm_comm_allreduce_sum(c, h->grad.p, h->grad.n, (void *)h->comm_stream));
    BM_HIP(hipEventRecord(h->ev_reduced[s], h->comm_stream));
    return 0;
}
int bm_rbm_wait_grads(bm_rbm *h, int32_t slot) {
    BM_CHECK(h && (slot == 0 || slot == 1) && h->comm_stream, "no reduction was started on slot %d", slot);
    BM_HIP(hipStreamWaitEvent(h->stream, h->ev_reduced[slot], 0));
    return 0;
}

int bm_rbm_apply_step(bm_rbm *h, int32_t B_global, float lr, float mom) {
    BM_TRY(check_dw(h, "bm_rbm_apply_step"));
    ProfScope _ps(h, KC_BIAS);
    RbmBiasArgs b;
    fill_bias(h, (float)B_global, lr, mom, b);
    ApplyWArgs a;
    memset(&a, 0, sizeof(a));
    a.raw = h->grad.p; a.raw2 = nullptr;
    a.W = h->W.p; a.dW = h->dW.p; a.Wt = nullptr;
    h->wt_valid = false;
    a.I = h->H; a.J = h->V; a.ldw = h->W.ld; a.ldwt = 0; a.form = 0;
    a.N = (float)B_global; a.M = a.N; a.l2 = h->cfg.l2; a.lr = lr; a.mom = mom;
    if (h->cfg.sparsity_cost != 0.f) {
        hipLaunchKernelGGL(rbm_bias_kernel, dim3((h->V + h->H + 255) / 256), dim3(256), 0, h->stream, b);
        a.pen = h->pen.p;
        launch_apply_w(a, nullptr, h->stream);
    } else {
        a.pen = nullptr;
        launch_apply_w(a, &b, h->stream);
    }
    BM_HIP(hipGetLastError());
    return 0;
}

int bm_rbm_transform(bm_rbm *h, const float *X_dev, int32_t B, int32_t k, float *H_dev) {
    BM_CHECK(H_dev, "null output");
    BM_TRY(run_chain(h, X_dev, B, k, H_dev));
    h->call++;
    BM_HIP(hipGetLastError());
    return 0;
}

int bm_rbm_metrics(bm_rbm *h, const float *X_dev, int32_t B, int32_t k, float *out4) {
    BM_TRY(run_chain(h, X_dev, B, k, nullptr, true, false, false, true));
    BM_TRY(metrics_from_chain(h, B, out4));
    h->call++;
    return 0;
}
// ... 113 lines not shown
    BM_CHECK(n_steps >= 1, "n_steps must be >= 1");
    struct FastScope { bm_rbm *h; ~FastScope() { h->fast_now = false; } } fast_scope{h};
    const bool fast = h->fast && h->cfg.v_unit == BM_UNIT_BERNOULLI && !h->multinomial() && h->cfg.sample_v_states &&
                      h->cfg.sample_h_states && h->cfg.dropout < 0.f;
    if (!fast && !h->multinomial()) {
        ensure_wt(h);
        chain_begin(h);
        for (int t = 0; t < n_steps; ++t) {
            const bool first = t == 0, last = t == n_steps - 1;
            launch_down(h, first ? H_dev : h->hs.p, first ? h->H : h->hs.ld, B, nullptr, last ? V_dev : h->vs.p,
                        last ? h->V : h->vs.ld, h->cfg.sample_v_states, SITE_V, t);
            launch_up(h, last ? V_dev : h->vs.p, last ? h->V : h->vs.ld, B, nullptr, last ? H_dev : h->hs.p,
                      last ? h->H : h->hs.ld, h->cfg.sample_h_states, SITE_H, t);
        }
        BM_TRY(chain_end(h));
        h->call++;
        BM_HIP(hipGetLastError());
        return 0;
    }
    hipLaunchKernelGGL(copy2d_kernel, dim3(256), dim3(256), 0, h->stream, (const float *)H_dev, h->H, h->hs.p, h->hs.ld, B, h->H);
    if (fast) {
        if (!h->nonbinary.p) {
            BM_TRY(h->W3.alloc(3, h->V, h->H)); BM_TRY(h->W3t.alloc(3, h->H, h->V));
            BM_TRY(h->hs16.alloc(1, h->maxB, h->H)); BM_TRY(h->vs16.alloc(1, h->maxB, h->V));
            BM_TRY(h->nonbinary.alloc(1));
            BM_HIP(hipMemsetAsync(h->nonbinary.p, 0, sizeof(int), h->stream));
        }
        hipLaunchKernelGGL(split3_kernel, dim3(512), dim3(256), 0, h->stream, (const float *)h->W.p, h->W.ld, h->V, h->H,
                           h->W3.p, h->W3.plane_stride(), h->W3.ld, 0);
        hipLaunchKernelGGL(split3_kernel, dim3(512), dim3(256), 0, h->stream, (const float *)h->W.p, h->W.ld, h->V, h->H,
                           h->W3t.p, h->W3t.plane_stride(), h->W3t.ld, 1);
        hipLaunchKernelGGL(shadow16_check_kernel, dim3(256), dim3(256), 0, h->stream, (const float *)h->hs.p, h->hs.ld, B, h->H,
                           h->hs16.p, h->hs16.ld, h->nonbinary.p);
        h->fast_now = true;
    }
    for (int t = 0; t < n_steps; ++t) {
        launch_down(h, h->hs.p, h->hs.ld, B, nullptr, h->vs.p, h->vs.ld, h->cfg.sample_v_states, SITE_V, t);
        launch_up(h, h->vs.p, h->vs.ld, B, nullptr, h->hs.p, h->hs.ld, h->cfg.sample_h_states, SITE_H, t);
    }
    hipLaunchKernelGGL(copy2d_kernel, dim3(256), dim3(256), 0, h->stream, (const float *)h->hs.p, h->hs.ld, H_dev, h->H, B, h->H);
    hipLaunchKernelGGL(copy2d_kernel, dim3(256), dim3(256), 0, h->stream, (const float *)h->vs.p, h->vs.ld, V_dev, h->V, B, h->V);
    h->call++;
    BM_HIP(hipGetLastError());
    return 0;
}

int bm_debug_tile_map(int32_t tiles_i, int32_t tiles_j, double bytes_i, double bytes_j, int32_t *out_ti, int32_t *out_tj,
                      int32_t *out_map5) {
    BM_CHECK(tiles_i >= 1 && tiles_j >= 1 && out_ti && out_tj, "bad arguments");
    const TileMap m = make_tile_map(tiles_i, tiles_j, bytes_i, bytes_j);
    const int nb = tiles_i * tiles_j;
    for (int b = 0; b < nb; ++b) { int ti = -1, tj = -1; tile_of_block(m, b, nb, ti, tj); out_ti[b] = ti; out_tj[b] = tj; }
    if (out_map5) { out_map5[0] = m.xi; out_map5[1] = m.xj; out_map5[2] = m.gj; out_map5[3] = m.tiles_i; out_map5[4] = m.tiles_j; }
    return 0;
}

int bm_rbm_stream(bm_rbm *h, void **out_stream) { *out_stream = (void *)h->stream; return 0; }

int bm_rbm_profile(bm_rbm *h, int32_t enable) {
    BM_HIP(hipStreamSynchronize(h->stream));
    h->recs.clear();
    h->prof = enable != 0;
    return 0;
}

int bm_rbm_kernel_times(bm_rbm *h, float *ms6, int32_t *n6) {
    BM_HIP(hipStreamSynchronize(h->stream));
    for (int c = 0; c < BM_NUM_KERNEL_CLASSES; ++c) { ms6[c] = 0.f; n6[c] = 0; }
    for (auto &r : h->recs) {
        float ms = 0.f;
        BM_HIP(hipEventElapsedTime(&ms, r.a, r.b));
        ms6[r.cls] += ms;
        n6[r.cls] += 1;
    }
    return 0;
}

int bm_rbm_chain_stats(bm_rbm *h, int64_t *out3) {
    BM_CHECK(h && out3, "null argument");
    out3[0] = (int64_t)h->chain.launches; out3[1] = (int64_t)h->chain.tiles_expected; out3[2] = (int64_t)chain_mode(h->chain);
    return 0;
}

int bm_rbm_timer_start(bm_rbm *h) { BM_HIP(hipEventRecord(h->ev0, h->stream)); return 0; }
int bm_rbm_timer_mark(bm_rbm *h) { BM_HIP(hipEventRecord(h->ev1, h->stream)); return 0; }
int bm_rbm_timer_elapsed(bm_rbm *h, float *out_ms) {
    BM_HIP(hipEventSynchronize(h->ev1));
    BM_HIP(hipEventElapsedTime(out_ms, h->ev0, h->ev1));
    return 0;
}
int bm_rbm_timer_stop(bm_rbm *h, float *out_ms) {
    BM_HIP(hipEventRecord(h->ev1, h->stream));
    BM_HIP(hipEventSynchronize(h->ev1));
    BM_HIP(hipEventElapsedTime(out_ms, h->ev0, h->ev1));
    return 0;
}

}
```

### boltzmann_machines_amd/engine.py

```python
import ctypes as C

import numpy as np

from . import _ffi
from ._ffi import DeviceArray, check

RBM_VARS = ('W', 'vb', 'hb', 'dW', 'dvb', 'dhb', 'q_means', 'sigma')


def as_device(X):
    if isinstance(X, DeviceArray):
        return X
    return DeviceArray.from_numpy(np.asarray(X), np.float32)


class RbmEngine(object):
    dtype = np.float32

    def __init__(self, n_visible, n_hidden, v_unit=_ffi.UNIT_BERNOULLI, sample_v_states=False,
                 sample_h_states=True, dbm_first=False, dbm_last=False, max_batch=10, l2=1e-4,
                 sparsity_target=0.1, sparsity_cost=0., sparsity_damping=0.9, dropout=None,
                 h_unit=_ffi.UNIT_BERNOULLI, n_samples=0):
        self.lib = _ffi.load()
        self.V, self.H, self.max_batch = int(n_visible), int(n_hidden), int(max_batch)
# ... 59 lines not shown
        check(self.lib.bm_rbm_set_row_offset(self._h, int(row0)))

    def sync(self):
        check(self.lib.bm_rbm_sync(self._h))

    def train_step(self, Xd, B, lr, momentum, k, row=0):
        check(self.lib.bm_rbm_train_step(self._h, Xd.offset_ptr(row * self.V), B, lr, momentum, k))

    def train_step_metrics(self, Xd, B, lr, momentum, k, row=0):
        out = (C.c_float * 4)()
        check(self.lib.bm_rbm_train_step_metrics(self._h, Xd.offset_ptr(row * self.V), B, lr, momentum, k, out))
        return np.array(out[:], dtype=np.float32)

    MAX_PENDING_METRICS = 4096

    def train_step_metrics_async(self, Xd, B, lr, momentum, k, row=0):
        check(self.lib.bm_rbm_train_step_metrics_async(self._h, Xd.offset_ptr(row * self.V), B, lr, momentum, k))

    def collect_metrics(self):
        out = np.empty((self.MAX_PENDING_METRICS, 4), dtype=np.float32)
        n = C.c_int32(0)
        check(self.lib.bm_rbm_collect_metrics(self._h, out.ctypes.data_as(C.POINTER(C.c_float)),
                                              self.MAX_PENDING_METRICS, C.byref(n)))
        return out[:n.value].copy()

    def train_epoch(self, Xd, N, batch, lr, momentum, k, row=0):
        check(self.lib.bm_rbm_train_epoch(self._h, Xd.offset_ptr(row * self.V), N, batch, lr, momentum, k))

    def grad_step(self, Xd, B, k, row=0):
        check(self.lib.bm_rbm_grad_step(self._h, Xd.offset_ptr(row * self.V), B, k))

    def apply_step(self, B_global, lr, momentum):
        check(self.lib.bm_rbm_apply_step(self._h, B_global, lr, momentum))

    def set_grad_slot(self, slot):
        check(self.lib.bm_rbm_set_grad_slot(self._h, slot))

    def allreduce_grads_async(self, comm):
        check(self.lib.bm_rbm_allreduce_grads_async(self._h, comm._c))

    def wait_grads(self, slot):
        check(self.lib.bm_rbm_wait_grads(self._h, slot))

    def transform(self, Xd, B, k, Hd, row=0, out_row=0):
        check(self.lib.bm_rbm_transform(self._h, Xd.offset_ptr(row * self.V), B, k, Hd.offset_ptr(out_row * self.H)))

    def metrics(self, Xd, B, k, row=0):
        out = (C.c_float * 4)()
        check(self.lib.bm_rbm_metrics(self._h, Xd.offset_ptr(row * self.V), B, k, out))
        return np.array(out[:], dtype=np.float32)

    def free_energy(self, Xd, B, row=0):
        out = C.c_float()
        check(self.lib.bm_rbm_free_energy(self._h, Xd.offset_ptr(row * self.V), B, C.byref(out)))
        return float(out.value)

    def free_energy_rows(self, Xd, B, row=0):
        out = np.empty(B, dtype=np.float32)
        check(self.lib.bm_rbm_free_energy_rows(self._h, Xd.offset_ptr(row * self.V), B, out.ctypes.data_as(C.c_void_p)))
        return out

    def ais(self, n_betas, n_runs, k, seed, chain0=0, base_bias=None):
        out = np.empty(n_runs, dtype=np.float32)
        a = None
        if base_bias is not None:
            a = np.ascontiguousarray(base_bias, dtype=np.float32)
            if a.shape != (self.V,):
                raise ValueError('base_bias has shape %r, expected (%d,)' % (a.shape, self.V))
        check(self.lib.bm_rbm_ais(self._h, n_betas, n_runs, k, a.ctypes.data_as(C.c_void_p) if a is not None else None,
                                  int(seed), int(chain0), out.ctypes.data_as(C.c_void_p)))
        return out

    def gibbs(self, Hd, Vd, B, n_steps):
        check(self.lib.bm_rbm_gibbs(self._h, Hd.ptr, Vd.ptr, B, n_steps))

    def stream(self):
        p = C.c_void_p()
        check(self.lib.bm_rbm_stream(self._h, C.byref(p)))
        return p.value

    def chain_stats(self):
        out = (C.c_int64 * 3)()
        check(self.lib.bm_rbm_chain_stats(self._h, out))
        return int(out[0]), int(out[1]), int(out[2])

    def profile(self, enable):
        check(self.lib.bm_rbm_profile(self._h, int(bool(enable))))

    def kernel_times(self):
        ms, n = (C.c_float * 6)(), (C.c_int32 * 6)()
        check(self.lib.bm_rbm_kernel_times(self._h, ms, n))
        names = ('act_up', 'act_down', 'grad', 'colsum', 'bias', 'other')
        return {k: (float(ms[i]), int(n[i])) for i, k in enumerate(names)}

    def timer_start(self):
        check(self.lib.bm_rbm_timer_start(self._h))

    def timer_stop(self):
        ms = C.c_float()
        check(self.lib.bm_rbm_timer_stop(self._h, C.byref(ms)))
        return float(ms.value)

    def timer_mark(self):
        check(self.lib.bm_rbm_timer_mark(self._h))

    def timer_elapsed(self):
        ms = C.c_float()
        check(self.lib.bm_rbm_timer_elapsed(self._h, C.byref(ms)))
        return float(ms.value)


class RbmEngine64(object):

    dtype = np.float64

    def __init__(self, n_visible, n_hidden, v_unit=_ffi.UNIT_BERNOULLI, sample_v_states=False,
                 sample_h_states=True, dbm_first=False, dbm_last=False, max_batch=10, l2=1e-4,
                 sparsity_target=0.1, sparsity_cost=0., sparsity_damping=0.9, dropout=None,
                 h_unit=_ffi.UNIT_BERNOULLI, n_samples=0):
        self.lib = _ffi.load()
        self.V, self.H, self.max_batch = int(n_visible), int(n_hidden), int(max_batch)
        drop = -1.0 if dropout is None else float(dropout)
        cfg = _ffi.RbmConfig(self.V, self.H, int(v_unit), int(bool(sample_v_states)),
                             int(bool(sample_h_states)), int(bool(dbm_first)), int(bool(dbm_last)),
                             self.max_batch, float(l2), float(sparsity_target), float(sparsity_cost),
                             float(sparsity_damping), drop, int(h_unit), int(n_samples))
        hyper = (C.c_double * 5)(float(l2), float(sparsity_target), float(sparsity_cost), float(sparsity_damping), drop)
        self._h = C.c_void_p()
        check(self.lib.bm_rbm64_create(C.byref(cfg), hyper, C.byref(self._h)))

    def close(self):
        if getattr(self, '_h', None) is not None and self._h:
            self.lib.bm_rbm64_destroy(self._h)
            self._h = None

    def __del__(self):
        try:
            self.close()
        except Exception:
            pass

    def _shape(self, name):
        if name in ('W', 'dW'):
            return (self.V, self.H)
        return (self.V,) if name in ('vb', 'dvb', 'sigma') else (self.H,)

    def set(self, name, value):
        a = np.ascontiguousarray(np.broadcast_to(np.asarray(value, dtype=np.float64), self._shape(name)))
        check(self.lib.bm_rbm64_set_param(self._h, name.encode(), a.ctypes.data_as(C.c_void_p), a.size))

    def get(self, name):
        a = np.empty(self._shape(name), dtype=np.float64)
        check(self.lib.bm_rbm64_get_param(self._h, name.encode(), a.ctypes.data_as(C.c_void_p), a.size))
        return a

    def seed(self, seed):
        check(self.lib.bm_rbm64_seed(self._h, int(seed) & 0xFFFFFFFFFFFFFFFF))

    def set_row_offset(self, row0):
        check(self.lib.bm_rbm64_set_row_offset(self._h, int(row0)))

    def sync(self):
        check(self.lib.bm_rbm64_sync(self._h))

    def train_step(self, Xd, B, lr, momentum, k, row=0):
        check(self.lib.bm_rbm64_train_step(self._h, Xd.offset_ptr(row * self.V), B, lr, momentum, k))
# ... 287 lines not shown
```

### include/bm355.h

```cpp
#ifndef BM355_H
#define BM355_H

#include <stddef.h>
#include <stdint.h>

#ifdef __cplusplus
extern "C" {
#endif

const char *bm_last_error(void);
const char *bm_version(void);
int bm_device_count(void);
int bm_set_device(int device);

int bm_dev_alloc(size_t bytes, void **out_dev);
int bm_dev_free(void *dev);
int bm_h2d(void *dst_dev, const void *src_host, size_t bytes);
int bm_d2h(void *dst_host, const void *src_dev, size_t bytes);
int bm_dev_memset(void *dst_dev, int value, size_t bytes);

int bm_debug_tile_map(int32_t tiles_i, int32_t tiles_j, double bytes_i, double bytes_j, int32_t *out_ti,
                      int32_t *out_tj, int32_t *out_map5);

typedef struct bm_rbm bm_rbm;

enum { BM_UNIT_BERNOULLI = 0, BM_UNIT_GAUSSIAN = 1, BM_UNIT_MULTINOMIAL = 2 };

typedef struct bm_rbm_config {
    int32_t n_visible;
    int32_t n_hidden;
    int32_t v_unit;
    int32_t sample_v_states;
    int32_t sample_h_states;
    int32_t dbm_first;
    int32_t dbm_last;
    int32_t max_batch;
    float   l2;
    float   sparsity_target;
    float   sparsity_cost;
    float   sparsity_damping;
    float   dropout;
    int32_t h_unit;
    int32_t n_samples;
} bm_rbm_config;

int bm_rbm_create(const bm_rbm_config *cfg, bm_rbm **out);
int bm_rbm_destroy(bm_rbm *h);
int bm_rbm_sync(bm_rbm *h);

int bm_rbm_set_param(bm_rbm *h, const char *name, const float *host, size_t n);
int bm_rbm_set_param_dev(bm_rbm *h, const char *name, const float *src_dev, size_t n);
int bm_rbm_get_param(bm_rbm *h, const char *name, float *host, size_t n);
int bm_rbm_dev_ptr(bm_rbm *h, const char *name, void **out_dev, size_t *out_n);

int bm_rbm_seed(bm_rbm *h, uint64_t seed);
int bm_rbm_set_row_offset(bm_rbm *h, int64_t row0);

int bm_rbm_train_step(bm_rbm *h, const float *X_dev, int32_t B,
                      float learning_rate, float momentum, int32_t n_gibbs_steps);
int bm_rbm_train_step_metrics(bm_rbm *h, const float *X_dev, int32_t B,
                              float learning_rate, float momentum, int32_t n_gibbs_steps,
                              float *out4);
int bm_rbm_train_step_metrics_async(bm_rbm *h, const float *X_dev, int32_t B,
                                    float learning_rate, float momentum, int32_t n_gibbs_steps);
int bm_rbm_collect_metrics(bm_rbm *h, float *out4n, int32_t max_n, int32_t *out_n);
int bm_rbm_train_epoch(bm_rbm *h, const float *X_dev, int64_t N, int32_t batch,
                       float learning_rate, float momentum, int32_t n_gibbs_steps);

int bm_rbm_stage(bm_rbm *h, int32_t slot);
int bm_rbm_get_staged(bm_rbm *h, int32_t slot, const char *name, float *host, size_t n);

int bm_rbm_grad_step(bm_rbm *h, const float *X_dev, int32_t B_local, int32_t n_gibbs_steps);
int bm_rbm_apply_step(bm_rbm *h, int32_t B_global, float learning_rate, float momentum);

int bm_rbm_transform(bm_rbm *h, const float *X_dev, int32_t B, int32_t n_gibbs_steps,
                     float *H_dev);

int bm_rbm_metrics(bm_rbm *h, const float *X_dev, int32_t B, int32_t n_gibbs_steps,
                   float *out4);
int bm_rbm_free_energy(bm_rbm *h, const float *X_dev, int32_t B, float *out1);
int bm_rbm_free_energy_rows(bm_rbm *h, const float *X_dev, int32_t B, float *out_host);
int bm_rbm_ais(bm_rbm *h, int32_t n_betas, int32_t n_runs, int32_t n_gibbs_steps, const float *base_bias_host,
               uint64_t seed, int64_t chain0, float *values_host);

int bm_rbm_gibbs(bm_rbm *h, float *H_dev, float *V_dev, int32_t B, int32_t n_steps);

int bm_rbm_stream(bm_rbm *h, void **out_stream);

#define BM_NUM_KERNEL_CLASSES 6
int bm_rbm_profile(bm_rbm *h, int32_t enable);
int bm_rbm_kernel_times(bm_rbm *h, float *ms6, int32_t *n6);

int bm_rbm_chain_stats(bm_rbm *h, int64_t *out3);

int bm_rbm_timer_start(bm_rbm *h);
int bm_rbm_timer_stop(bm_rbm *h, float *out_ms);
int bm_rbm_timer_mark(bm_rbm *h);
int bm_rbm_timer_elapsed(bm_rbm *h, float *out_ms);

typedef struct bm_rbm64 bm_rbm64;
int bm_rbm64_create(const bm_rbm_config *cfg, const double *hyper5, bm_rbm64 **out);
int bm_rbm64_destroy(bm_rbm64 *h);
int bm_rbm64_sync(bm_rbm64 *h);
int bm_rbm64_seed(bm_rbm64 *h, uint64_t seed);
int bm_rbm64_set_row_offset(bm_rbm64 *h, int64_t row0);
int bm_rbm64_set_param(bm_rbm64 *h, const char *name, const double *host, size_t n);
int bm_rbm64_get_param(bm_rbm64 *h, const char *name, double *host, size_t n);
int bm_rbm64_train_step(bm_rbm64 *h, const double *X_dev, int32_t B,
                        double learning_rate, double momentum, int32_t n_gibbs_steps);
int bm_rbm64_train_step_metrics(bm_rbm64 *h, const double *X_dev, int32_t B,
                                double learning_rate, double momentum, int32_t n_gibbs_steps, double *out4);
int bm_rbm64_transform(bm_rbm64 *h, const double *X_dev, int32_t B, int32_t n_gibbs_steps,
                       double *H_dev);
int bm_rbm64_metrics(bm_rbm64 *h, const double *X_dev, int32_t B, int32_t n_gibbs_steps,
                     double *out4);
int bm_rbm64_free_energy(bm_rbm64 *h, const double *X_dev, int32_t B, double *out1);


typedef struct bm_dbm bm_dbm;

#define BM_DBM_MAX_LAYERS 4

typedef struct bm_dbm_config {
    int32_t n_layers;
    int32_t n_visible;
    int32_t n_hiddens[BM_DBM_MAX_LAYERS];
    int32_t v_unit;
    int32_t sample_v_states;
    int32_t sample_h_states[BM_DBM_MAX_LAYERS];
    int32_t n_particles;
    int32_t batch_size;
    int32_t max_mf_updates;
    float   mf_tol;
    float   l2;
    float   max_norm;
    float   sparsity_target[BM_DBM_MAX_LAYERS];
    float   sparsity_cost[BM_DBM_MAX_LAYERS];
    float   sparsity_damping;
    int32_t h_unit[BM_DBM_MAX_LAYERS];
    int32_t n_samples[BM_DBM_MAX_LAYERS];
} bm_dbm_config;

int bm_dbm_create(const bm_dbm_config *cfg, bm_dbm **out);
int bm_dbm_destroy(bm_dbm *h);
int bm_dbm_sync(bm_dbm *h);
int bm_dbm_seed(bm_dbm *h, uint64_t seed);
int bm_dbm_set_row_offset(bm_dbm *h, int64_t row0, int64_t particle0);

int bm_dbm_set_param(bm_dbm *h, const char *name, const float *host, size_t n);
int bm_dbm_get_param(bm_dbm *h, const char *name, float *host, size_t n);
int bm_dbm_dev_ptr(bm_dbm *h, const char *name, void **out_dev, size_t *out_n);

int bm_dbm_train_step(bm_dbm *h, const float *X_dev, float learning_rate, float momentum,
                      int32_t n_gibbs_steps, int32_t *out_n_mf, float *out_msre);
int bm_dbm_metrics(bm_dbm *h, const float *X_dev, int32_t n_gibbs_steps, int32_t *out_n_mf, float *out_msre);
int bm_dbm_grad_step(bm_dbm *h, const float *X_dev, int32_t n_gibbs_steps, int32_t *out_n_mf);
int bm_dbm_apply_step(bm_dbm *h, int32_t N_global, int32_t M_global,
                      float learning_rate, float momentum);
int bm_dbm_set_mf_allreduce(bm_dbm *h, float (*fn)(float local_max, void *ctx), void *ctx);
int bm_dbm_stream(bm_dbm *h, void **out_stream);

int bm_dbm_mean_field(bm_dbm *h, const float *X_dev, float *MU_top_dev, int32_t *out_n_mf);
int bm_dbm_reconstruct(bm_dbm *h, const float *X_dev, float *R_dev);
int bm_dbm_sample_v(bm_dbm *h, int32_t n_gibbs_steps, float *V_dev);
int bm_dbm_ais(bm_dbm *h, int32_t n_betas, int32_t n_runs, int32_t n_gibbs_steps,
               uint64_t seed, int64_t chain0, float *values_host);
int bm_dbm_log_proba(bm_dbm *h, const float *X_dev, float *out_host);

int bm_dbm_timer_start(bm_dbm *h);
int bm_dbm_timer_stop(bm_dbm *h, float *out_ms);
int bm_dbm_timer_mark(bm_dbm *h);
int bm_dbm_timer_elapsed(bm_dbm *h, float *out_ms);


typedef struct bm_comm bm_comm;
int bm_comm_unique_id(void *out_id128);
// ... 67 lines not shown
```

Before: 15850.

## Fuse weight update with next batch's hidden-layer pass in one linked kernel

```diff
diff --git a/boltzmann_machines_amd/_ffi.py b/boltzmann_machines_amd/_ffi.py
--- a/boltzmann_machines_amd/_ffi.py
+++ b/boltzmann_machines_amd/_ffi.py
@@ -137,6 +137,8 @@
     'bm_rbm_profile': [_vp, _i32],
     'bm_rbm_kernel_times': [_vp, _fp, _ip],
     'bm_rbm_chain_stats': [_vp, C.POINTER(C.c_int64)],
+    'bm_rbm_link_stats': [_vp, C.POINTER(C.c_int64)],
+    'bm_rbm_set_link': [_vp, C.c_int32],
     'bm_rbm_timer_start': [_vp],
     'bm_rbm_timer_stop': [_vp, _fp],
     'bm_rbm_timer_mark': [_vp],
diff --git a/boltzmann_machines_amd/csrc/bm_chain.h b/boltzmann_machines_amd/csrc/bm_chain.h
--- a/boltzmann_machines_amd/csrc/bm_chain.h
+++ b/boltzmann_machines_amd/csrc/bm_chain.h
@@ -194,16 +194,20 @@
     }
 };
 
+static inline bool team_device_ok(int &ncu) {
+    hipDeviceProp_t pr; int d = 0, nxcc = 0; (void)hipGetDevice(&d);
+    const bool have = hipGetDeviceProperties(&pr, d) == hipSuccess;
+    ncu = have ? pr.multiProcessorCount : 0;
+    if (hipDeviceGetAttribute(&nxcc, hipDeviceAttributeNumberOfXccs, d) != hipSuccess) nxcc = 0;
+    const bool arch = have && (strncmp(pr.gcnArchName, "gfx950", 6) == 0 || strncmp(pr.gcnArchName, "gfx942", 6) == 0);
+    return arch && nxcc == 8 && ncu == 256;
+}
+
 static inline int chain_mode(ChainState &cs) {
     if (cs.mode < 0) {
         const char *e = bm::dbg("chain");
         cs.mode = e ? atoi(e) : 1;
-        hipDeviceProp_t pr; int d = 0, nxcc = 0; (void)hipGetDevice(&d);
-        const bool have = hipGetDeviceProperties(&pr, d) == hipSuccess;
-        cs.ncu = have ? pr.multiProcessorCount : 0;
-        if (hipDeviceGetAttribute(&nxcc, hipDeviceAttributeNumberOfXccs, d) != hipSuccess) nxcc = 0;
-        const bool arch = have && (strncmp(pr.gcnArchName, "gfx950", 6) == 0 || strncmp(pr.gcnArchName, "gfx942", 6) == 0);
-        if (!(arch && nxcc == 8 && cs.ncu == 256)) cs.mode = 0;
+        if (!team_device_ok(cs.ncu)) cs.mode = 0;
     }
     return cs.mode;
 }
diff --git a/boltzmann_machines_amd/csrc/bm_gemm.h b/boltzmann_machines_amd/csrc/bm_gemm.h
--- a/boltzmann_machines_amd/csrc/bm_gemm.h
+++ b/boltzmann_machines_amd/csrc/bm_gemm.h
@@ -9,8 +9,10 @@
 struct NoSide {
     static constexpr bool kFinalSync = true;
     static constexpr bool kSplitFill = false, kCohQ = false;
+    static constexpr bool kWaitP = false, kCohP = false;
     static constexpr bool kCanAbort = false;
     __device__ __forceinline__ void wait_inputs() {}
+    __device__ __forceinline__ void post_wait() {}
     __device__ __forceinline__ void post_fill() {}
     __device__ __forceinline__ void fill() {}
     __device__ __forceinline__ void drain() {}
@@ -327,10 +329,13 @@
     asm volatile("s_mov_b32 m0, %2\n\ts_nop 0\n\tglobal_load_lds_dwordx4 %1, %0 sc1"
                  :: "s"(sbase), "v"(voff), "s"(lds_byte) : "memory");
 }
-template <class G, int DW, bool QSC = false, bool QHALF = false>
+template <class G, int DW, bool QSC = false, bool QHALF = false, bool PSC = false>
 __device__ __forceinline__ void dma_chunk_s(const DmaPlan<G, DW> &pl, const char *pb, const char *qb, unsigned ldsP, unsigned ldsQ) {
 #pragma unroll
-    for (int n = 0; n < DmaPlan<G, DW>::NPP; ++n) dma16s(pb, pl.p[n], ldsP + (unsigned)(n * DW * 1024));
+    for (int n = 0; n < DmaPlan<G, DW>::NPP; ++n) {
+        if (PSC) dma16s_coh(pb, pl.p[n], ldsP + (unsigned)(n * DW * 1024));
+        else     dma16s(pb, pl.p[n], ldsP + (unsigned)(n * DW * 1024));
+    }
 #pragma unroll
     for (int n = 0; n < DmaPlan<G, DW>::NPQ; ++n) {
         if (QHALF && (n & 1)) continue;
@@ -366,17 +371,17 @@
     }
 }
 
-template <int QL, class G, bool FAST, bool SEG2, int PL = KM, bool COHQ = false>
+template <int QL, class G, bool FAST, bool SEG2, int PL = KM, bool COHQ = false, bool COHP = false>
 __device__ __forceinline__ void load_chunk(ChunkRegs<G> &r, const KRange &kr, int nch1, int i0, int j0, int c, int tid) {
     constexpr int BK = G::BK;
     if (!SEG2) {
-        g2r<PL, G::TI, BK, G::NT, FAST>(r.p, kr.P1.ptr, kr.P1.ld, kr.P1.nx, kr.P1.vec, i0, c * BK, kr.K1, tid);
+        g2r<PL, G::TI, BK, G::NT, FAST, COHP>(r.p, kr.P1.ptr, kr.P1.ld, kr.P1.nx, kr.P1.vec, i0, c * BK, kr.K1, tid);
         g2r<QL, G::TJ, BK, G::NT, FAST, COHQ>(r.q, kr.Q1.ptr, kr.Q1.ld, kr.Q1.nx, kr.Q1.vec, j0, c * BK, kr.K1, tid);
     } else {
         const int m = -(int)((c >= nch1) & (kr.K2 > 0));
         const int kc = c - (nch1 & m);
         const int K = sel_i(kr.K1, kr.K2, m);
-        g2r<PL, G::TI, BK, G::NT, FAST>(r.p, sel_p(kr.P1.ptr, kr.P2.ptr, m), sel_i(kr.P1.ld, kr.P2.ld, m),
+        g2r<PL, G::TI, BK, G::NT, FAST, COHP>(r.p, sel_p(kr.P1.ptr, kr.P2.ptr, m), sel_i(kr.P1.ld, kr.P2.ld, m),
                                         sel_i(kr.P1.nx, kr.P2.nx, m), sel_i(kr.P1.vec, kr.P2.vec, m), i0, kc * BK, K, tid);
         g2r<QL, G::TJ, BK, G::NT, FAST, COHQ>(r.q, sel_p(kr.Q1.ptr, kr.Q2.ptr, m), sel_i(kr.Q1.ld, kr.Q2.ld, m),
                                               sel_i(kr.Q1.nx, kr.Q2.nx, m), sel_i(kr.Q1.vec, kr.Q2.vec, m), j0, kc * BK, K, tid);
@@ -523,6 +528,28 @@
         static_assert(FAST && STG == STG_DMA && DW == G::NW, "chained fill");
         const unsigned l0 = (unsigned)(uintptr_t)(__attribute__((address_space(3))) void *)smem;
         const unsigned lP = l0 + (unsigned)w * 1024u, lQ = l0 + (unsigned)(NBUF * P_BUF * 4) + (unsigned)w * 1024u;
+        if constexpr (Side::kWaitP) {
+#pragma unroll
+            for (int c = 0; c < PF; ++c) {
+                const char *qb = (const char *)kr.Q1.ptr + (size_t)c * ((QL == KM) ? (size_t)BK * kr.Q1.ld * 4 : (size_t)BK * 4);
+#pragma unroll
+                for (int n = 0; n < DmaPlan<G, DW>::NPQ; ++n) dma16s(qb, pl1.q[n], lQ + (unsigned)(c * Q_BUF * 4 + n * DW * 1024));
+            }
+            __builtin_amdgcn_sched_barrier(0);
+            side.fill();
+            __builtin_amdgcn_sched_barrier(0);
+            side.wait_inputs();
+            side.post_wait();
+            __builtin_amdgcn_sched_barrier(0);
+#pragma unroll
+            for (int c = 0; c < PF; ++c) {
+                const char *pb = (const char *)kr.P1.ptr + (size_t)c * ((PL == KM) ? (size_t)BK * kr.P1.ld * 4 : (size_t)BK * 4);
+#pragma unroll
+                for (int n = 0; n < DmaPlan<G, DW>::NPP; ++n) dma16s_coh(pb, pl1.p[n], lP + (unsigned)(c * P_BUF * 4 + n * DW * 1024));
+            }
+            constexpr int NP_LEFT = (PF - 2) * DmaPlan<G, DW>::NPP;
+            BM_WAIT_VM(NP_LEFT);
+        } else {
 #pragma unroll
         for (int c = 0; c < PF; ++c) {
             const char *pb = (const char *)kr.P1.ptr + (size_t)c * ((PL == KM) ? (size_t)BK * kr.P1.ld * 4 : (size_t)BK * 4);
@@ -541,6 +568,7 @@
         }
         constexpr int NQ_LEFT = (PF - 2) * DmaPlan<G, DW>::NPQ;
         BM_WAIT_VM(NQ_LEFT);
+        }
     } else {
 #pragma unroll
         for (int c = 0; c < PF; ++c)
@@ -610,7 +638,7 @@
         if (SEG2 && !in2 && (CD) >= nch1) { in2 = true; pl1 = pl2; }                              \
         const char *pb_, *qb_;                                                                    \
         chunk_bases((CD), pb_, qb_);                                                              \
-        if (dmaw) dma_chunk_s<G, DW, Side::kCohQ, (BM_ABL(9) != 0)>(pl1, pb_, qb_, ldsPw + (unsigned)((SD) * P_BUF * 4), \
+        if (dmaw) dma_chunk_s<G, DW, Side::kCohQ, (BM_ABL(9) != 0), Side::kCohP>(pl1, pb_, qb_, ldsPw + (unsigned)((SD) * P_BUF * 4), \
                                      ldsQw + (unsigned)((SD) * Q_BUF * 4));                       \
     }
 #define BM_STEP_Q(FC, FN, S)                                                                      \
@@ -629,7 +657,7 @@
         const bool do_dma = cd < nch && is_dma(cd) && !BM_ABL(0);                                 \
         const bool do_reg = cr < nch && !is_dma(cr) && !BM_ABL(0);                                \
         if (cc == last - 1) side.drain();       \
-        if (do_reg) load_chunk<QL, G, FAST, SEG2, PL, Side::kCohQ>(gr, kr, nch1, i0, j0, cr, tid); \
+        if (do_reg) load_chunk<QL, G, FAST, SEG2, PL, Side::kCohQ, Side::kCohP>(gr, kr, nch1, i0, j0, cr, tid); \
         if (do_dma) BM_DMA_AT(cd, S3)                                                             \
         read_frags<QL, G, ABL, PL>(FN, sP + (S1) * P_BUF, sQ + (S1) * Q_BUF, wi, wj, lane);       \
         mfma_frags<G, ABL>(acc, FC);                                                              \
diff --git a/boltzmann_machines_amd/csrc/bm_kernels.h b/boltzmann_machines_amd/csrc/bm_kernels.h
--- a/boltzmann_machines_amd/csrc/bm_kernels.h
+++ b/boltzmann_machines_amd/csrc/bm_kernels.h
@@ -150,6 +150,7 @@
 template <int E, class Rng, bool MF = false, int NTH = 256> struct ActSide {
     static constexpr bool kFinalSync = false;
     static constexpr bool kSplitFill = false, kCohQ = false, kCanAbort = MF;
+    static constexpr bool kWaitP = false, kCohP = false;
     static constexpr bool kMF = MF;
     const float *bias, *sigma;
     const float *prev_row;
@@ -749,6 +750,7 @@
 template <int NJ> struct GradSide {
     static constexpr bool kFinalSync = true;
     static constexpr bool kSplitFill = false, kCohQ = false, kCanAbort = false;
+    static constexpr bool kWaitP = false, kCohP = false;
     const float *W, *dW; int ldw, I, J, ib0, jb[NJ]; bool on, vec8;
     float4 w[NJ][2], d[NJ][2];
     bool at_fill;
@@ -778,33 +780,9 @@
     }
 };
 
-template <class G, bool FAST, int ABL = 0, int STG = STG_DMA, int MINB = 1>
-__global__ __launch_bounds__(G::NT, MINB) void grad_kernel(GradArgs a, TileMap tmap) {
-    constexpr int TI = G::TI, NJ = G::NJ;
-    static_assert(G::MI == 2 && G::TI == 64 && G::TJ == 64, "grad_kernel: 64 x 64 tiles, 8 consecutive outputs per lane");
-    __shared__ __attribute__((aligned(16))) float smem[G::SMEM_FLOATS];
-    constexpr bool kBias = G::SMEM_FLOATS >= CS_SMEM_FLOATS;
-    static_assert(G::NT >= NT, "bias path");
-    const int ntile_blocks = (int)gridDim.x - a.nbias;
-    if ((int)blockIdx.x >= ntile_blocks) {
-        if constexpr (kBias) {
-            if (G::NT > NT && threadIdx.x >= NT) return;
-            rbm_bias_fused_block(a.bias, (int)blockIdx.x - ntile_blocks, smem);
-        }
-        return;
-    }
-    asm volatile("" :: "s"(a.Ppos.ptr), "s"(a.Qpos.ptr), "s"(a.Ppos.ld), "s"(a.Qpos.ld), "s"(a.Ppos.nx), "s"(a.Qpos.nx),
-                       "s"(a.Pneg.ptr), "s"(a.Qneg.ptr), "s"(a.Pneg.ld), "s"(a.Qneg.ld), "s"(a.Kpos), "s"(a.Kneg),
-                       "s"(a.I), "s"(a.J), "s"(a.W), "s"(a.dW), "s"(a.ldw), "s"(a.form), "s"(a.fused));
-    constexpr int TJ2 = G::TJ;
-    int ti, tj;
-    if (tmap.slab) {
-        block_to_tile((a.J + TJ2 - 1) / TJ2, ti, tj, 0, a.nbias);
-    } else {
-        TILE_WORDS(tmap, (int)blockIdx.x);
-        TILE_OF_BLOCK(tmap, (int)blockIdx.x, ntile_blocks, ti, tj);
-    }
-    const int i0 = ti * TI, j0 = tj * TJ2;
+template <class G, bool FAST, int ABL, int STG>
+__device__ __forceinline__ void grad_tile(const GradArgs &a, int i0, int j0, float *smem) {
+    constexpr int NJ = G::NJ;
     const int tid = threadIdx.x, lane = tid & 63, w = tid >> 6;
     const int wi = w % G::WI, wj = w / G::WI;
     const int g = lane >> 4, l15 = lane & 15;
@@ -911,6 +889,35 @@
         }
     }
     BM_GSTAMP(2);
+}
+
+template <class G, bool FAST, int ABL = 0, int STG = STG_DMA, int MINB = 1>
+__global__ __launch_bounds__(G::NT, MINB) void grad_kernel(GradArgs a, TileMap tmap) {
+    constexpr int TI = G::TI;
+    static_assert(G::MI == 2 && G::TI == 64 && G::TJ == 64, "grad_kernel: 64 x 64 tiles, 8 consecutive outputs per lane");
+    __shared__ __attribute__((aligned(16))) float smem[G::SMEM_FLOATS];
+    constexpr bool kBias = G::SMEM_FLOATS >= CS_SMEM_FLOATS;
+    static_assert(G::NT >= NT, "bias path");
+    const int ntile_blocks = (int)gridDim.x - a.nbias;
+    if ((int)blockIdx.x >= ntile_blocks) {
+        if constexpr (kBias) {
+            if (G::NT > NT && threadIdx.x >= NT) return;
+            rbm_bias_fused_block(a.bias, (int)blockIdx.x - ntile_blocks, smem);
+        }
+        return;
+    }
+    asm volatile("" :: "s"(a.Ppos.ptr), "s"(a.Qpos.ptr), "s"(a.Ppos.ld), "s"(a.Qpos.ld), "s"(a.Ppos.nx), "s"(a.Qpos.nx),
+                       "s"(a.Pneg.ptr), "s"(a.Qneg.ptr), "s"(a.Pneg.ld), "s"(a.Qneg.ld), "s"(a.Kpos), "s"(a.Kneg),
+                       "s"(a.I), "s"(a.J), "s"(a.W), "s"(a.dW), "s"(a.ldw), "s"(a.form), "s"(a.fused));
+    constexpr int TJ2 = G::TJ;
+    int ti, tj;
+    if (tmap.slab) {
+        block_to_tile((a.J + TJ2 - 1) / TJ2, ti, tj, 0, a.nbias);
+    } else {
+        TILE_WORDS(tmap, (int)blockIdx.x);
+        TILE_OF_BLOCK(tmap, (int)blockIdx.x, ntile_blocks, ti, tj);
+    }
+    grad_tile<G, FAST, ABL, STG>(a, ti * TI, tj * TJ2, smem);
 }
 
 struct ApplyWArgs {
diff --git a/boltzmann_machines_amd/csrc/bm_link.h b/boltzmann_machines_amd/csrc/bm_link.h
--- /dev/null
+++ b/boltzmann_machines_amd/csrc/bm_link.h
@@ -0,0 +1,240 @@
+#pragma once
+#include "bm_chain.h"
+
+namespace bm {
+
+using GeoLinkG = GeoGrad8;
+using GeoLinkA = GeoAct8;
+constexpr int LINK_FLAGS = 64;
+static_assert(GeoLinkG::NT == GeoLinkA::NT && GeoLinkG::SMEM_FLOATS >= GeoLinkA::SMEM_FLOATS && GeoLinkG::SMEM_FLOATS >= CS_SMEM_FLOATS,
+              "one workgroup shape and one LDS image for the three kinds of job");
+
+struct LinkArgs {
+    GradArgs g;
+    Operand P, Q; int K, I, J;
+    const float *bias; float mult, bmult;
+    float *means, *states; int ldo;
+    PhiloxKey key; long long row0;
+    int ncb, ntj, nvb, tiles_j;
+    unsigned gen;
+    unsigned *flags;
+    unsigned *claim, *claim_zero;
+    int *status;
+};
+static_assert(sizeof(LinkArgs) <= 4096, "kernel arguments");
+
+template <int E, class Rng> struct LinkSide : ActSide<E, Rng> {
+    static constexpr bool kSplitFill = true, kWaitP = true, kCohP = true, kCohQ = false, kCanAbort = false;
+    const unsigned *wflags;
+    int nwait;
+    unsigned gen;
+    int *status;
+    __device__ __forceinline__ void fill() { if (this->with_rng) this->rng.fill(); }
+    __device__ __forceinline__ void wait_inputs() {
+        if ((threadIdx.x >> 6) == 0) {
+            const int lane = threadIdx.x & 63;
+            unsigned spins = 0;
+            for (;;) {
+                unsigned v = gen;
+                if (lane < nwait) v = __hip_atomic_load(wflags + lane, __ATOMIC_RELAXED, __HIP_MEMORY_SCOPE_AGENT);
+                if (__all(v == gen)) break;
+                __builtin_amdgcn_s_sleep(1);
+                if ((++spins & 1023u) == 0) {
+                    const int st = __hip_atomic_load(status, __ATOMIC_RELAXED, __HIP_MEMORY_SCOPE_AGENT);
+                    if (st || spins > (1u << 21)) {
+                        if (lane == 0 && !st) atomicExch(status, CHAIN_ERR_TIMEOUT);
+                        break;
+                    }
+                }
+            }
+        }
+        wg_barrier();
+    }
+    __device__ __forceinline__ void post_wait() {
+#pragma unroll
+        for (int e = 0; e < E; ++e) {
+            const int i = (this->ib0 + e < this->I) ? this->ib0 + e : this->I - 1;
+            this->bs[e] = __uint_as_float(__hip_atomic_load(reinterpret_cast<const unsigned *>(this->bias) + i, __ATOMIC_RELAXED, __HIP_MEMORY_SCOPE_AGENT));
+            this->sg[e] = 1.0f;
+        }
+    }
+};
+
+__device__ __forceinline__ void link_h0_tile(const LinkArgs &c, int i0, int j0, float *smem, const unsigned *wflags, int nwait) {
+    using G = GeoLinkA;
+    constexpr int E = G::E;
+    ActArgs a;
+    a.P1 = c.P; a.Q1 = c.Q; a.K1 = c.K; a.p_xm = 1;
+    a.P2 = Operand{nullptr, 0, 0, 0}; a.Q2 = a.P2; a.K2 = 0;
+    a.I = c.I; a.J = c.J;
+    a.bias = c.bias; a.sigma = nullptr; a.mult = c.mult; a.bmult = c.bmult; a.kind = 0; a.sample = 1;
+    a.means = c.means; a.states = c.states; a.negmeans = nullptr; a.ldo = c.ldo;
+    a.key = c.key; a.row0 = c.row0;
+    a.prev = nullptr; a.maxdiff = nullptr; a.maxdiff_blk = nullptr;
+    a.rowacc = nullptr; a.beta_a = 0.f; a.beta_b = 0.f; a.rowacc_single = 0; a.rowdot_out = nullptr; a.ld_part = 0;
+    a.dot_vec = nullptr; a.dot_mat = nullptr; a.ld_dot = 0;
+    a.acc_init = nullptr; a.ld_init = 0; a.skip = nullptr;
+    a.chk_ctl = nullptr; a.chk_slots = nullptr; a.chk_n = 0; a.chk_tol = 0.f;
+    a.b3 = Bf3Range{}; a.states16 = nullptr; a.ld16 = 0; a.map_xi = 0;
+    a.fe_rowacc2 = nullptr; a.fe_flip = nullptr; a.fe_x = nullptr; a.fe_ldx = 0; a.fe_w = nullptr; a.fe_ldw = 0;
+    a.fe_zero = nullptr; a.fe_rm = 0; a.fe_key = PhiloxKey{0u, 0u, 0u, 0u};
+#ifdef BM_PROBE
+    a.dbg = nullptr;
+#endif
+    const int tid = threadIdx.x, lane = tid & 63, w = tid >> 6;
+    const int wi = w % G::WI, wj = w / G::WI;
+    const int g = lane >> 4, l15 = lane & 15;
+    const int ib0 = i0 + wi * (16 * G::MI) + g * E;
+    const int j = j0 + wj * 16 + l15;
+    KRange kr;
+    kr.P1 = a.P1; kr.Q1 = a.Q1; kr.K1 = a.K1;
+    kr.P2 = a.P2; kr.Q2 = a.Q2; kr.K2 = 0;
+    LinkSide<E, typename PhiloxFor<G::MI>::type> side;
+    side.bias = a.bias; side.sigma = nullptr; side.ib0 = ib0; side.I = a.I; side.with_rng = 1;
+    side.prev_row = nullptr;
+    side.wflags = wflags; side.nwait = nwait; side.gen = c.gen; side.status = c.status;
+    const PhiloxKey key = a.key;
+    side.rng.init(key, ((unsigned long long)(a.row0 + j) * (unsigned long long)a.I + ib0) >> 2);
+    f32x4 acc[G::MI][1];
+#pragma unroll
+    for (int t = 0; t < G::MI; ++t) acc[t][0] = (f32x4){0.f, 0.f, 0.f, 0.f};
+    mainloop<XM, G, true, false, 0, XM, STG_DMA>(acc, kr, i0, j0, smem, side);
+    (void)act_epilogue<G, 0>(a, key, acc, side, i0, j0);
+}
+
+__global__ __launch_bounds__(GeoLinkG::NT, 1) void link_kernel(LinkArgs c) {
+    __shared__ __attribute__((aligned(16))) float smem[GeoLinkG::SMEM_FLOATS];
+    __shared__ unsigned s_claim;
+    const int tid = threadIdx.x;
+    unsigned xcc_reg;
+    asm volatile("s_getreg_b32 %0, hwreg(HW_REG_XCC_ID)" : "=s"(xcc_reg));
+    const int team = (int)(xcc_reg & 7u);
+    if ((xcc_reg & 0xfu) > 7u) {
+        if (tid == 0) atomicExch(c.status, CHAIN_ERR_XCC);
+        return;
+    }
+    if (blockIdx.x == 0 && tid < 8) c.claim_zero[tid * 32] = 0u;
+    unsigned *my_claim = c.claim + team * 32;
+    if (tid == 0) s_claim = __hip_atomic_fetch_add(my_claim, 1u, __ATOMIC_RELAXED, __HIP_MEMORY_SCOPE_AGENT);
+    __syncthreads();
+    int n = (int)s_claim;
+    wg_barrier();
+    const int nc = (c.ncb - team + 7) >> 3, nvt = (c.nvb - team + 7) >> 3;
+    const int n_tiles = nc * c.ntj, n_hb = n_tiles + nc, n_vb = n_hb + nvt, n_all = n_vb + nc * 2 * c.tiles_j;
+    const int nbar = 2 * ((c.g.bias.B + CS_ROWS - 1) / CS_ROWS);
+    int njobs = 0;
+    while (n < n_all) {
+        unsigned *flag = nullptr;
+        if (n < n_tiles) {
+            const int q = small_div(n, c.ntj), tj = n - q * c.ntj, cb = team + 8 * q;
+            grad_tile<GeoLinkG, true, 0, STG_DMA>(c.g, cb * GeoLinkG::TI, tj * GeoLinkG::TJ, smem);
+            flag = c.flags + (size_t)cb * LINK_FLAGS + tj;
+        } else if (n < n_vb) {
+            const bool hid = n < n_hb;
+            const int cb = team + 8 * (hid ? n - n_tiles : n - n_hb);
+            if (tid < NT) rbm_bias_fused_block(c.g.bias, hid ? c.nvb + cb : cb, smem);
+            else for (int b = 0; b < nbar; ++b) wg_barrier();
+            if (hid) flag = c.flags + (size_t)cb * LINK_FLAGS + c.ntj;
+        } else {
+            const int m = n - n_vb, per = 2 * c.tiles_j;
+            const int q = small_div(m, per), r = m - q * per, cb = team + 8 * q;
+            const int i0 = cb * 64 + (r & 1) * GeoLinkA::TI, j0 = (r >> 1) * GeoLinkA::TJ;
+            if (i0 < c.I) link_h0_tile(c, i0, j0, smem, c.flags + (size_t)cb * LINK_FLAGS, c.ntj + 1);
+        }
+        asm volatile("s_waitcnt vmcnt(0)" ::: "memory");
+        if (tid == 0) s_claim = __hip_atomic_fetch_add(my_claim, 1u, __ATOMIC_RELAXED, __HIP_MEMORY_SCOPE_AGENT);
+        wg_barrier();
+        if (tid == 0 && flag) __hip_atomic_store(flag, c.gen, __ATOMIC_RELAXED, __HIP_MEMORY_SCOPE_AGENT);
+        n = (int)s_claim;
+        wg_barrier();
+        ++njobs;
+    }
+    if (tid == 0 && njobs) atomicAdd(c.status + 1, njobs);
+}
+
+struct LinkState {
+    unsigned *flags = nullptr, *claim = nullptr;
+    int *status = nullptr;
+    int ncb_cap = 0;
+    unsigned gen = 0;
+    unsigned launches = 0;
+    long long jobs_expected = 0;
+    int mode = -1;
+    int ncu = 0;
+    static constexpr int CLAIM_SLOTS = 16;
+    LinkState() = default;
+    LinkState(const LinkState &) = delete;
+    LinkState &operator=(const LinkState &) = delete;
+    ~LinkState() {
+        if (flags) (void)hipFree(flags);
+        if (claim) (void)hipFree(claim);
+        if (status) (void)hipFree(status);
+    }
+};
+
+static inline int link_mode(LinkState &ls) {
+    if (ls.mode < 0) {
+        const char *e = bm::dbg("link");
+        ls.mode = e ? atoi(e) : 0;
+        if (!team_device_ok(ls.ncu)) ls.mode = 0;
+    }
+    return ls.mode;
+}
+
+static inline bool link_ok(const LinkState &ls, const GradArgs &g, const ActArgs &a) {
+    using GA = GeoLinkA;
+    if (!(g.fused && g.form == 0 && g.Wt && g.nbias > 0 && !g.pen)) return false;
+    if (!(operand_fast(g.Ppos, KM, g.Kpos) && operand_fast(g.Qpos, KM, g.Kpos) && operand_fast(g.Pneg, KM, g.Kneg) &&
+          operand_fast(g.Qneg, KM, g.Kneg))) return false;
+    if (!(a.p_xm && a.P1.ptr == g.Wt && a.kind == 0 && a.sample && a.K2 == 0 && a.I == g.I && a.K1 == g.J)) return false;
+    if (!(operand_fast(a.P1, XM, a.K1) && operand_fast(a.Q1, XM, a.K1))) return false;
+    if (a.K1 < GA::PF * GA::BK) return false;
+    if ((g.J + 63) / 64 + 1 > LINK_FLAGS) return false;
+    if (ls.mode == 1) {
+        const int ncb = (g.I + 63) / 64, ntj = (g.J + 63) / 64;
+        if (ncb < 8 || ncb * ntj > ls.ncu) return false;
+    }
+    return true;
+}
+
+static inline int link_launch(LinkState &ls, hipStream_t st, const GradArgs &g, const ActArgs &a) {
+    const int ncb = (g.I + 63) / 64, ntj = (g.J + 63) / 64;
+    if (!ls.flags || ncb > ls.ncb_cap) {
+        if (ls.flags) { if (hipStreamSynchronize(st) != hipSuccess) return -1; (void)hipFree(ls.flags); ls.flags = nullptr; }
+        const size_t nfl = (size_t)ncb * LINK_FLAGS;
+        if (hipMalloc((void **)&ls.flags, nfl * 4) != hipSuccess) return -1;
+        if (hipMemsetAsync(ls.flags, 0, nfl * 4, st) != hipSuccess) return -1;
+        ls.ncb_cap = ncb;
+        ls.gen = 0;
+        if (!ls.claim) {
+            if (hipMalloc((void **)&ls.claim, (size_t)LinkState::CLAIM_SLOTS * 8 * 32 * 4) != hipSuccess) return -1;
+            if (hipMemsetAsync(ls.claim, 0, (size_t)LinkState::CLAIM_SLOTS * 8 * 32 * 4, st) != hipSuccess) return -1;
+            if (hipMalloc((void **)&ls.status, 2 * sizeof(int)) != hipSuccess) return -1;
+            if (hipMemsetAsync(ls.status, 0, 2 * sizeof(int), st) != hipSuccess) return -1;
+        }
+    }
+    LinkArgs c;
+    memset(&c, 0, sizeof(c));
+    c.g = g;
+    c.g.fetch_at_fill = 0;
+    c.P = a.P1; c.Q = a.Q1; c.K = a.K1; c.I = a.I; c.J = a.J;
+    c.bias = a.bias; c.mult = a.mult; c.bmult = a.bmult;
+    c.means = a.means; c.states = a.states; c.ldo = a.ldo;
+    c.key = a.key; c.row0 = a.row0;
+    c.ncb = ncb; c.ntj = ntj; c.nvb = ntj; c.tiles_j = (a.J + GeoLinkA::TJ - 1) / GeoLinkA::TJ;
+    if (++ls.gen == 0) {
+        if (hipMemsetAsync(ls.flags, 0, (size_t)ls.ncb_cap * LINK_FLAGS * 4, st) != hipSuccess) return -1;
+        ls.gen = 1;
+    }
+    c.gen = ls.gen;
+    c.flags = ls.flags;
+    c.claim = ls.claim + (size_t)(ls.launches % LinkState::CLAIM_SLOTS) * 8 * 32;
+    c.claim_zero = ls.claim + (size_t)((ls.launches + LinkState::CLAIM_SLOTS / 2) % LinkState::CLAIM_SLOTS) * 8 * 32;
+    ++ls.launches;
+    c.status = ls.status;
+    ls.jobs_expected += (long long)ncb * ntj + ncb + ntj + (long long)ncb * 2 * c.tiles_j;
+    hipLaunchKernelGGL(link_kernel, dim3(ls.ncu), dim3(GeoLinkG::NT), 0, st, c);
+    return 0;
+}
+
+}
diff --git a/boltzmann_machines_amd/csrc/bm_rbm.hip b/boltzmann_machines_amd/csrc/bm_rbm.hip
--- a/boltzmann_machines_amd/csrc/bm_rbm.hip
+++ b/boltzmann_machines_amd/csrc/bm_rbm.hip
@@ -2,6 +2,7 @@
 #include "bm_common.h"
 #include "bm_kernels.h"
 #include "bm_chain.h"
+#include "bm_link.h"
 
 #include <math.h>
 #include <atomic>
@@ -89,6 +90,9 @@
     std::vector<Rec> recs;
     size_t grad_tail() const { return (size_t)V * W.ld; }
     ChainState chain;
+    LinkState link;
+    Mat h0m_alt, h0s_alt;
+    bool h0_ready = false;
 };
 
 enum { KC_UP = 0, KC_DOWN = 1, KC_GRAD = 2, KC_COLSUM = 3, KC_BIAS = 4, KC_OTHER = 5 };
@@ -224,7 +228,7 @@
 static bool metrics_fused_ok(const bm_rbm *h);
 static void metrics_prep(bm_rbm *h, int B);
 static int run_chain(bm_rbm *h, const float *X_dev, int B, int k, float *hm_out, bool need_vm = true, bool for_update = false,
-                     bool split_step = false, bool fetch = false) {
+                     bool split_step = false, bool fetch = false, bool have_h0 = false) {
     BM_CHECK(B >= 1 && B <= h->maxB, "batch %d outside [1, max_batch=%d]", B, h->maxB);
     BM_CHECK(k >= 1, "n_gibbs_steps must be >= 1 (got %d)", k);
     if (!split_step) ensure_wt(h);
@@ -247,7 +251,7 @@
     h->fe_in_chain = fe;
     if (fetch && !fe) metrics_prep(h, B);
     chain_begin(h);
-    launch_up(h, Xin, ldx, B, h->h0m.p, h->h0s.p, h->h0m.ld, 1, SITE_H0, 0, nullptr, fe);
+    if (!have_h0) launch_up(h, Xin, ldx, B, h->h0m.p, h->h0s.p, h->h0m.ld, 1, SITE_H0, 0, nullptr, fe);
     const float *hstate = h->cfg.sample_h_states ? h->h0s.p : h->h0m.p;
     for (int t = 0; t < k; ++t) {
         const bool last = t == k - 1;
@@ -612,6 +616,21 @@
                      "are invalid, chained launches are now off for this handle", (unsigned)st[1], expect);
         }
     }
+    if (h->link.status) {
+        int st[2] = {0, 0};
+        BM_HIP(hipMemcpy(st, h->link.status, sizeof(st), hipMemcpyDeviceToHost));
+        const long long expect = h->link.jobs_expected & 0xffffffffLL;
+        if (st[0] != 0 || (long long)(unsigned)st[1] != expect) {
+            h->link.mode = 0;
+            h->link.jobs_expected = 0;
+            BM_HIP(hipMemset(h->link.status, 0, sizeof(st)));
+            BM_CHECK(st[0] == 0, "linked update launch failed (status %d: %s); the results since the last check are invalid, "
+                     "linked launches are now off for this handle", st[0],
+                     st[0] == CHAIN_ERR_TIMEOUT ? "a wait for a producing tile expired" : "not an 8-XCD device");
+            BM_CHECK(false, "linked update launches ran %u jobs, expected %lld; the results since the last check are invalid, "
+                     "linked launches are now off for this handle", (unsigned)st[1], expect);
+        }
+    }
     return 0;
 }
 
@@ -737,6 +756,12 @@
         BM_CHECK(*(const int *)h->stage_host.h == 0, "a chained propagation launch failed (status %d) before this snapshot: "
                  "it is invalid (bm_rbm_sync reports and recovers)", *(const int *)h->stage_host.h);
     }
+    if (h->link.status) {
+        BM_HIP(hipMemcpyAsync(h->stage_host, h->link.status, sizeof(int), hipMemcpyDeviceToHost, h->stage_stream));
+        BM_HIP(hipStreamSynchronize(h->stage_stream));
+        BM_CHECK(*(const int *)h->stage_host.h == 0, "a linked update launch failed (status %d) before this snapshot: "
+                 "it is invalid (bm_rbm_sync reports and recovers)", *(const int *)h->stage_host.h);
+    }
     if (nm == "W" || nm == "dW") {
         BM_CHECK(n == (size_t)h->V * h->H, "variable '%s' has %zu elements, got %zu", name, (size_t)h->V * h->H, n);
         const Mat &m = nm == "W" ? sg.W : sg.dW;
@@ -815,7 +840,7 @@
     BM_CHECK(h && out_n && (out4n || max_n == 0), "null argument");
     BM_CHECK(h->mring_n <= max_n, "%d fetches pending, room for %d", h->mring_n, (int)max_n);
     if (h->mring_n > 0 && h->ev_mlast) BM_HIP(hipEventSynchronize(h->ev_mlast));
-    if (h->chain.status || h->xchg_used) {
+    if (h->chain.status || h->link.status || h->xchg_used) {
         BM_HIP(hipStreamSynchronize(h->stream));
         const int rc = check_device_status(h);
         if (rc) { h->mring_n = 0; *out_n = 0; return rc; }
@@ -826,11 +851,60 @@
     return 0;
 }
 
+static bool link_step_ok(bm_rbm *h) {
+    return link_mode(h->link) > 0 && h->cfg.sparsity_cost == 0.f && !h->multinomial() && h->use_wt && h->cfg.dropout < 0.f &&
+           h->cfg.v_unit == BM_UNIT_BERNOULLI && !h->fast_now && !h->prof;
+}
+static int update_linked(bm_rbm *h, int B, float lr, float mom, const float *Xn, int Bn, bool &linked) {
+    linked = false;
+    GradArgs g;
+    fill_grad(h, B, 1, (float)B, lr, mom, g);
+    g.pen = nullptr;
+    g.nbias = fill_bias_fused(h, B, lr, mom, g.bias);
+    g.bias.raw_only = 0;
+    if (!h->h0m_alt.p) { BM_TRY(h->h0m_alt.alloc(h->maxB, h->H)); BM_TRY(h->h0s_alt.alloc(h->maxB, h->H)); }
+    ActArgs a;
+    memset(&a, 0, sizeof(a));
+    a.P1 = make_operand(h->Wt.p, h->Wt.ld, h->H); a.p_xm = 1;
+    a.Q1 = make_operand(Xn, h->V, Bn);
+    a.K1 = h->V; a.I = h->H; a.J = Bn;
+    a.bias = h->hb.p;
+    a.mult = 1.0f + (h->cfg.dbm_first ? 1.0f : 0.0f); a.bmult = a.mult;
+    a.kind = BM_UNIT_BERNOULLI; a.sample = 1;
+    a.means = h->h0m_alt.p; a.states = h->h0s_alt.p; a.ldo = h->h0m_alt.ld;
+    a.key = make_key(h, SITE_H0, 0); a.key.call = h->call + 1;
+    a.row0 = h->row0;
+    if (!link_ok(h->link, g, a)) return 0;
+    BM_CHECK(link_launch(h->link, h->stream, g, a) == 0, "linked launch: %s", hipGetErrorString(hipGetLastError()));
+    h->wt_valid = true;
+    std::swap(h->h0m.p, h->h0m_alt.p);
+    std::swap(h->h0s.p, h->h0s_alt.p);
+    linked = true;
+    return 0;
+}
+
 int bm_rbm_train_epoch(bm_rbm *h, const float *X_dev, int64_t N, int32_t batch, float lr, float mom, int32_t k) {
     BM_CHECK(batch >= 1 && N >= 1, "bad N=%lld batch=%d", (long long)N, batch);
+    struct Scope { bm_rbm *h; ~Scope() { h->h0_ready = false; } } scope{h};
+    h->h0_ready = false;
     for (int64_t s = 0; s < N; s += batch) {
         const int B = (int)((N - s < batch) ? (N - s) : batch);
-        BM_TRY(bm_rbm_train_step(h, X_dev + (size_t)s * h->V, B, lr, mom, k));
+        const int64_t sn = s + batch;
+        const int Bn = sn < N ? (int)((N - sn < batch) ? (N - sn) : batch) : 0;
+        if (!(h->h0_ready || (Bn > 0 && link_step_ok(h)))) {
+            BM_TRY(bm_rbm_train_step(h, X_dev + (size_t)s * h->V, B, lr, mom, k));
+            continue;
+        }
+        BM_TRY(check_dw(h, "bm_rbm_train_epoch"));
+        const bool have_h0 = h->h0_ready;
+        h->h0_ready = false;
+        BM_TRY(run_chain(h, X_dev + (size_t)s * h->V, B, k, nullptr, false, true, false, false, have_h0));
+        bool linked = false;
+        if (Bn > 0 && link_step_ok(h)) BM_TRY(update_linked(h, B, lr, mom, X_dev + (size_t)sn * h->V, Bn, linked));
+        if (!linked) launch_update_fused(h, B, lr, mom);
+        h->h0_ready = linked;
+        h->call++;
+        BM_HIP(hipGetLastError());
     }
     return 0;
 }
@@ -1110,6 +1184,19 @@
     return 0;
 }
 
+int bm_rbm_set_link(bm_rbm *h, int32_t mode) {
+    BM_CHECK(h && mode >= 0 && mode <= 2, "link mode must be 0, 1 or 2");
+    (void)link_mode(h->link);
+    if (team_device_ok(h->link.ncu)) h->link.mode = mode;
+    return 0;
+}
+
+int bm_rbm_link_stats(bm_rbm *h, int64_t *out3) {
+    BM_CHECK(h && out3, "null argument");
+    out3[0] = (int64_t)h->link.launches; out3[1] = (int64_t)h->link.jobs_expected; out3[2] = (int64_t)link_mode(h->link);
+    return 0;
+}
+
 int bm_rbm_timer_start(bm_rbm *h) { BM_HIP(hipEventRecord(h->ev0, h->stream)); return 0; }
 int bm_rbm_timer_mark(bm_rbm *h) { BM_HIP(hipEventRecord(h->ev1, h->stream)); return 0; }
 int bm_rbm_timer_elapsed(bm_rbm *h, float *out_ms) {
diff --git a/boltzmann_machines_amd/engine.py b/boltzmann_machines_amd/engine.py
--- a/boltzmann_machines_amd/engine.py
+++ b/boltzmann_machines_amd/engine.py
@@ -165,6 +165,14 @@
     def chain_stats(self):
         out = (C.c_int64 * 3)()
         check(self.lib.bm_rbm_chain_stats(self._h, out))
+        return int(out[0]), int(out[1]), int(out[2])
+
+    def set_link(self, mode):
+        check(self.lib.bm_rbm_set_link(self._h, int(mode)))
+
+    def link_stats(self):
+        out = (C.c_int64 * 3)()
+        check(self.lib.bm_rbm_link_stats(self._h, out))
         return int(out[0]), int(out[1]), int(out[2])
 
     def profile(self, enable):
diff --git a/include/bm355.h b/include/bm355.h
--- a/include/bm355.h
+++ b/include/bm355.h
@@ -92,6 +92,9 @@
 int bm_rbm_kernel_times(bm_rbm *h, float *ms6, int32_t *n6);
 
 int bm_rbm_chain_stats(bm_rbm *h, int64_t *out3);
+
+int bm_rbm_link_stats(bm_rbm *h, int64_t *out3);
+int bm_rbm_set_link(bm_rbm *h, int32_t mode);
 
 int bm_rbm_timer_start(bm_rbm *h);
 int bm_rbm_timer_stop(bm_rbm *h, float *out_ms);
```

Result: slower. 15480 (-2.4%).
